# xuyuan/waymo_2d_tracking

Hardware: AMD Instinct MI355X
Metric: end-to-end frames/sec (detect+SORT) on 1920x1280 Waymo frames (higher is better)
Workload: dtype f32; 1 GPU; Cascade R-CNN X152-32x8d-FPN dconv (random-init, fp32, batch 1) on synthetic 1920x1280x3 frames -> top-100 detections/frame -> SORT (max_age 2, min_hits 0, all boxes tracked; trackers resident for the whole segment); 5 cameras x 2 frames per step per GPU; 1x1 and dense 3x3 convolutions: f32 operands as exact 3 x bf16 splits, six cross terms on the bf16 matrix cores, f32 accumulate (csrc/det_gemm_s; stage=e2e, parallelism=sequence-shard x1

## Files before the change

### include/waymodet.h

```cpp
#ifndef WAYMODET_H
#define WAYMODET_H
#include <stddef.h>
#include <stdint.h>
#ifdef __cplusplus
extern "C" {
#endif

int wd_roi_pool_fpn_f32(const float* const* feats, const int32_t* heights, const int32_t* widths,
                        const float* scales, int n_levels, int channels, int batch,
                        const float* rois, int n_rois, int pooled, int min_level, int canonical_level,
                        float canonical_size, float* out, void* stream);

size_t wd_nms_workspace(int n);
int wd_select_kept(const uint8_t* keep_mask, const uint8_t* valid, const int64_t* order, int n, int cap, int64_t* out_idx,
                   int32_t* count, void* stream);
int wd_nms_sorted_f32(const float* boxes, const int32_t* idxs, int n, float iou_threshold,
                      uint8_t* keep_mask, int32_t* n_keep, void* workspace, size_t workspace_bytes, void* stream);

size_t wd_gemm_nt_workspace(int M, int N, int K);
int wd_gemm_nt_ws_f32(const float* A, const float* Bt, const float* bias, const float* residual, int relu, int M, int N, int K,
                      float* C, void* workspace, size_t workspace_bytes, void* stream);

int wd_gemm_lt_f32(const float* a, const float* w, const float* bias, const float* residual, float* out, int m, int n, int k,
                   int relu, void* workspace, size_t workspace_bytes, void* stream);
int wd_gemm_lt_plan_info(int m, int n, int k, int relu, int has_bias, int has_residual, float* best_us, int* candidates);
size_t wd_gemm_split_packed_bytes(int N, int K);
int wd_gemm_split_pack_weight(const float* w, int N, int K, void* packed, void* stream);
int wd_gemm_split_pack_weight_strided(const float* w, int N, int K, long stride_n, long stride_k, void* packed, void* stream);
typedef struct WdSplitPackDesc {
    const float* src;
    void* dst;
    long s_n, s_c, s_kh, s_kw;
    long first_block;
    int N, K, C, ksize, flip, reserved;
} WdSplitPackDesc;
int wd_gemm_split_pack_batch(const WdSplitPackDesc* descs_device, int count, long total_blocks, void* stream);
size_t wd_gemm_split_workspace(long M, int N, int K);
int wd_gemm_split_f32(const float* a, long lda, const void* packed_w, const float* bias, const float* residual, float* out, long ldc,
                      int M, int N, int K, int relu, void* workspace, size_t workspace_bytes, void* stream);
int wd_conv_split_f32(const float* x, int batch, int H, int W, int C, const void* packed_w, int ksize, int stride, int pad, const float* bias,
                      const float* residual, float* out, int N, int relu, void* workspace, size_t workspace_bytes, void* stream);
int wd_gemm_split_supported(const float* a, long lda, const float* bias, const float* residual, const float* out, long ldc, long M, int N, int K);
int wd_conv_split_position_major(int batch, int H, int W, int ksize, int stride, int pad);
typedef struct WdSplitIO {
    const float* a;
    long lda;
    const void* a_planes;
    const float* residual;
    const void* residual_planes;
    float* out;
    void* out_planes;
    long ldc;
} WdSplitIO;
size_t wd_split_planes_bytes(long M, int K);
int wd_split_planes_pack_f32(const float* a, long lda, long M, int K, void* planes, void* stream);
int wd_split_planes_unpack_f32(const void* planes, long M, int K, float* out, long ldo, void* stream);
int wd_gemm_split_io(const WdSplitIO* io, const void* packed_w, const float* bias, int M, int N, int K, int relu, void* workspace,
                     size_t workspace_bytes, void* stream);
int wd_nms_segmented_f32(const float* boxes, const int32_t* idxs, const int32_t* seg_offsets, int n_seg, float iou_threshold,
                         uint8_t* keep_mask, int32_t* n_keep, void* workspace, size_t workspace_bytes, void* stream);

size_t wd_rpn_topk_workspace(const int* n_per_level, int n_levels, int k);
int wd_rpn_topk_decode_f32(const float* const* logits, const float* const* deltas, const float* const* anchors,
                           const int* n_per_level, int n_levels, int k, float img_h, float img_w, float scale_clamp,
                           float* out_boxes, float* out_scores, int32_t* out_group, uint8_t* out_valid, void* workspace,
                           size_t workspace_bytes, void* stream);
int wd_sort_candidates_f32(const float* boxes, const float* scores, const int32_t* group, const uint8_t* valid,
                           const uint8_t* valid2 , int n, float* out_boxes, float* out_scores, int32_t* out_group, uint8_t* out_valid, int64_t* out_order,
                           void* stream);
int wd_box_candidates_f32(const float* boxes, const float* s0, const float* s1, const float* s2, const int32_t* n_valid, int rows,
                          int num_classes, float score_thresh, float img_h, float img_w, float* out_boxes, float* out_scores,
                          int32_t* out_group, uint8_t* out_valid, int64_t* out_order, void* stream);
int wd_gather_kept_f32(const uint8_t* keep, const uint8_t* valid, const float* boxes, const float* scores, const int64_t* order,
                       int n, int cap, int num_classes, float* out_boxes, float* out_scores, int64_t* out_class, int32_t* count,
                       void* stream);
int wd_detections_to_wire(const float* boxes, const float* scores, const int64_t* classes, const int32_t* count, int n, int in_w,
                          int in_h, int hflip, int out_w, int out_h, double* xywhs, int32_t* category, void* stream);

size_t wd_deform_packed_weight_floats(int c_in, int c_out, int groups);
int wd_deform_pack_weight(const float* weight_oihw, int c_in, int c_out, int groups, float* packed, void* stream);
const char* wd_deform_conv3x3_variant(int c_in, int groups, int stride, int pad, int has_offset);
const char* wd_deform_conv3x3_last_kernel(void);
int wd_deform_conv3x3_f32(const float* x, const float* offset, const float* mask, const float* packed_weight,
                          const float* scale, const float* bias, int relu,
                          int batch, int h, int w, int c_in, int c_out, int groups, int stride, int pad,
                          float* y, void* stream);
int wd_deform_conv3x3_hint_f32(const float* x, const float* offset, const float* mask, const float* packed_weight,
                               const float* scale, const float* bias, int relu, int batch, int h, int w, int c_in,
                               int c_out, int groups, int stride, int pad, int far_offsets, float* y, void* stream);
size_t wd_deform_table_bytes(int batch, int h, int w);
int wd_deform_offsets_table_f32(const float* partial, int ld, const float* bias, int batch, int h, int w, float* offsets,
                                void* table, void* stream);
int wd_deform_conv3x3_tab_f32(const float* x, const float* offset, const float* mask, const float* packed_weight,
                              const float* scale, const float* bias, int relu, int batch, int h, int w, int c_in,
                              int c_out, int groups, int stride, int pad, int far_offsets, const void* table, float* y,
                              void* stream);

int wd_gemm_nt_f32(const float* A, const float* Bt, const float* bias, const float* residual, int relu,
                   int M, int N, int K, float* C, void* stream);

int wd_groupnorm_relu_nhwc_f32(float* x, const float* gamma, const float* beta, int n, int hw, int c, int groups,
                               float eps, int relu, void* stream);
int wd_groupnorm_relu_out_nhwc_f32(const float* x, float* y, const float* gamma, const float* beta, int n, int hw, int c, int groups,
                                   float eps, int relu, void* stream);
int wd_groupnorm_relu_bwd_nhwc_f32(const float* x, const float* dy, const float* gamma, const float* beta, int n, int hw, int c, int groups,
                                   float eps, int relu, float* dx, float* dgamma, float* dbeta, void* stream);

#define WD_LAYOUT_NCHW_F32 0
#define WD_LAYOUT_NHWC_U8 1
int wd_preprocess_out_shape(int h, int w, double scale, int divisor, int* ho, int* wo, int* hp, int* wp);
int wd_preprocess_f32(const void* src, int src_layout, int batch, int h, int w, double scale, int hflip, int vflip,
                      int swap_rb, const float* mean3, const float* std3, int divisor, float* out, void* stream);

int wd_decode_boxes_f32(const float* deltas, const float* boxes, const int64_t* index, int n, float wx, float wy, float ww,
                        float wh, float scale_clamp, float clip_w, float clip_h, float* out, void* stream);

int wd_roi_pool_fpn_bwd_f32(float* const* grad_feats, const int32_t* heights, const int32_t* widths, const float* scales,
                            int n_levels, int channels, int batch, const float* rois, int n_rois, int pooled, int min_level,
                            int canonical_level, float canonical_size, const float* grad_out, void* stream);
int wd_deform_im2col_f32(const float* x, const float* offset, int batch, int h, int w, int c, int groups, int stride, int pad,
                         float* col, void* stream);
int wd_deform_col2im_f32(const float* dcol, const float* x, const float* offset, int batch, int h, int w, int c, int groups,
                         int stride, int pad, float* dx, float* doffset, void* stream);
size_t wd_deform_bwd_tables_bytes(int batch, int h, int w, int stride);
int wd_deform_dxoff_f32(const float* x, const float* offset, const float* dy, const float* y_act, const float* scale, const float* weight, int batch,
                        int h, int w, int c, int groups, int stride, unsigned char* tables, float* packed_weight, float* dx, float* doffset,
                        void* stream);
size_t wd_deform_dw_scratch_floats(int batch, int h, int w, int c, int groups, int stride);
int wd_deform_dw_f32(const float* x, const float* offset, const float* dy, const float* y_act, const float* scale, int batch, int h, int w, int c,
                     int groups, int stride, float* scratch, float* dw, void* stream);

int wd_tap_shift_add_f32(const float* partial, int ld, int n_out, const float* bias, int batch, int h, int w, int stride,
                         float* out, void* stream);

int wd_upsample2x_nhwc_f32(const float* src, int batch, int h, int w, int c, float* dst, void* stream);

int wd_bias_relu_f32(float* y, const float* bias, long m, int n, int relu, void* stream);

int wd_act_bwd_f32(const float* dy, const float* y, const float* scale, long m, int n, int relu, float* g, void* stream);

int wd_autocontrast_u8(uint8_t* img, int h, int w, void* workspace24, void* stream);

int wd_jpeg_info(const uint8_t* data, int64_t n, int32_t* width, int32_t* height, int32_t* components, int32_t* h_samp,
                 int32_t* v_samp, int32_t* restart_interval);
int wd_jpeg_decode_rgb_u8(const uint8_t* data, int64_t n, uint8_t* rgb, int64_t capacity, int32_t* width, int32_t* height,
                          int32_t* sync_rounds, void* stream);
int wd_jpeg_last_stats(int32_t* out4);

#ifdef __cplusplus
}
#endif
#endif
```

### waymo_2d_tracking_amd/csrc/det_deform.hip

```cpp
#include "common.h"
#include "../../include/waymodet.h"
#include <cstdlib>

namespace {

using f32x4 = __attribute__((ext_vector_type(4))) float;
constexpr int TP = 64;
constexpr int CCH = 128;
constexpr int LDC = CCH + 2;

struct Sample {
    unsigned idx[4];
    float wgt[4];
};

template <int CG, bool DEFORM>
__global__ __launch_bounds__(256, (CG <= 32 ? 3 : 2)) void deform_conv3x3_kernel(
    const float* __restrict__ x, const float* __restrict__ offset, const float* __restrict__ mask,
    const float* __restrict__ wp, const float* __restrict__ scale, const float* __restrict__ bias, int relu,
    int batch, int H, int W, int C, int Cout, int Ho, int Wo, int stride, int pad, float* __restrict__ y) {
    constexpr bool PRIV = CG <= 32;
    constexpr int LDW = PRIV ? 34 : LDC;
    __shared__ Sample tab[TP * 9];
    __shared__ __attribute__((aligned(16))) float col[PRIV ? 4 * TP * 34 : TP * LDC];
    const int tid = threadIdx.x, lane = tid & 63, wave = tid >> 6;
    const int tiles_x = (Wo + 7) >> 3, tiles_y = (Ho + 7) >> 3;
    const int ntiles = batch * tiles_y * tiles_x;
    const int nchunks = C / CCH;
    int tile, chunk;
    {
        const int b = blockIdx.x;
        const int xcd = b & 7, slot = b >> 3;
        if (nchunks >= 8 && (nchunks & 7) == 0) {
            const int cpx = nchunks >> 3;
            chunk = xcd * cpx + slot % cpx;
            tile = slot / cpx;
        } else if (nchunks < 8 && (8 % nchunks) == 0 && (ntiles % (8 / nchunks)) == 0) {
            const int xpc = 8 / nchunks;
            const int tpp = ntiles / xpc;
            chunk = xcd / xpc;
            tile = (xcd % xpc) * tpp + slot;
        } else {
            chunk = b / ntiles;
            tile = b - chunk * ntiles;
        }
    }
    if (tile >= ntiles || chunk >= nchunks) return;
    const int tn = tile / (tiles_y * tiles_x);
    const int trem = tile - tn * tiles_y * tiles_x;
    const int tyy = trem / tiles_x, txx = trem - tyy * tiles_x;
    __shared__ int pix[TP];
    if (tid < TP) {
        const int ho = tyy * 8 + (tid >> 3), wo = txx * 8 + (tid & 7);
        pix[tid] = (ho < Ho && wo < Wo) ? (tn * Ho + ho) * Wo + wo : -1;
    }
    __syncthreads();
    const int c0 = chunk * CCH;
    for (int e = tid; e < TP * 9; e += 256) {
        const int p = e / 9, k = e - 9 * p;
        const long gp = pix[p];
        Sample s;
#pragma unroll
        for (int q = 0; q < 4; ++q) { s.idx[q] = 0u; s.wgt[q] = 0.f; }
        if (gp >= 0) {
            const int n = (int)(gp / ((long)Ho * Wo));
            const int rem = (int)(gp - (long)n * Ho * Wo);
            const int ho = rem / Wo, wo = rem - ho * Wo;
            const int kh = k / 3, kw = k - 3 * kh;
            if (!DEFORM) {
                const int hi = ho * stride - pad + kh, wi = wo * stride - pad + kw;
                if (hi >= 0 && hi < H && wi >= 0 && wi < W) { s.idx[0] = (unsigned)(n * H * W + hi * W + wi) * (unsigned)C * 4u; s.wgt[0] = 1.f; }
                tab[e] = s;
                continue;
            }
            const float* off = offset + (size_t)gp * 18;
            const float h_im = (float)(ho * stride - pad + kh) + off[2 * k];
            const float w_im = (float)(wo * stride - pad + kw) + off[2 * k + 1];
            if (h_im > -1.f && w_im > -1.f && h_im < (float)H && w_im < (float)W) {
                const int hl = (int)floorf(h_im), wl = (int)floorf(w_im);
                const int hh = hl + 1, wh = wl + 1;
                const float lh = h_im - (float)hl, lw = w_im - (float)wl;
                const float uh = 1.f - lh, uw = 1.f - lw;
                const float m = mask ? mask[(size_t)gp * 9 + k] : 1.f;
                const int base = n * H * W;
                if (hl >= 0 && wl >= 0) { s.idx[0] = (unsigned)(base + hl * W + wl) * (unsigned)C * 4u; s.wgt[0] = uh * uw * m; }
                if (hl >= 0 && wh <= W - 1) { s.idx[1] = (unsigned)(base + hl * W + wh) * (unsigned)C * 4u; s.wgt[1] = uh * lw * m; }
                if (hh <= H - 1 && wl >= 0) { s.idx[2] = (unsigned)(base + hh * W + wl) * (unsigned)C * 4u; s.wgt[2] = lh * uw * m; }
                if (hh <= H - 1 && wh <= W - 1) { s.idx[3] = (unsigned)(base + hh * W + wh) * (unsigned)C * 4u; s.wgt[3] = lh * lw * m; }
            }
        }
        tab[e] = s;
    }
    f32x4 acc[4][2];
#pragma unroll
    for (int i = 0; i < 4; ++i)
#pragma unroll
        for (int j = 0; j < 2; ++j) acc[i][j] = (f32x4){0.f, 0.f, 0.f, 0.f};
    __syncthreads();

    const int gq = PRIV ? (lane & 7) : (tid & 31);
    const int gp0 = PRIV ? (lane >> 3) : (tid >> 5);
    const int co_w = wave * 32;
    float* colw = PRIV ? col + wave * (TP * 34) : col;
    auto slab_sync = [&]() {
        if (PRIV) {
            __builtin_amdgcn_fence(__ATOMIC_RELEASE, "wavefront");
            __builtin_amdgcn_wave_barrier();
            __builtin_amdgcn_fence(__ATOMIC_ACQUIRE, "wavefront");
        } else {
            __syncthreads();
        }
    };
    constexpr int NQ = DEFORM ? 4 : 1;
    const char* xb = reinterpret_cast<const char*>(x);
    const unsigned lane_off = (unsigned)(c0 + (PRIV ? co_w : 0) + gq * 4) * 4u;
    float4 tA[4][NQ];
    auto issue = [&](int k, int half, float4 (&t)[4][NQ]) {
#pragma unroll
        for (int i = 0; i < 4; ++i) {
            const int p = gp0 + 8 * (half * 4 + i);
            const Sample& s = tab[p * 9 + k];
#pragma unroll
            for (int q = 0; q < NQ; ++q)
                t[i][q] = *reinterpret_cast<const float4*>(xb + (size_t)(s.idx[q] + lane_off));
        }
    };
    auto blend = [&](int k, int half, const float4 (&t)[4][NQ]) {
#pragma unroll
        for (int i = 0; i < 4; ++i) {
            const int p = gp0 + 8 * (half * 4 + i);
            const Sample& s = tab[p * 9 + k];
            float4 v = make_float4(0.f, 0.f, 0.f, 0.f);
#pragma unroll
            for (int q = 0; q < NQ; ++q) {
                const float wq = s.wgt[q];
                v.x += wq * t[i][q].x; v.y += wq * t[i][q].y;
                v.z += wq * t[i][q].z; v.w += wq * t[i][q].w;
            }
            float2* d = reinterpret_cast<float2*>(&colw[p * LDW + gq * 4]);
            d[0] = make_float2(v.x, v.y);
            d[1] = make_float2(v.z, v.w);
        }
    };
    constexpr int KS = (CG >= 16) ? CG / 4 : 4;
    float bR[2][KS];
    auto load_b = [&](int k) {
#pragma unroll
        for (int nt = 0; nt < 2; ++nt) {
            const int co_l = co_w + 16 * nt;
            if (CG >= 16) {
                const int g = (c0 + co_l) / CG;
                const int co_g = (co_l % CG) + (lane & 15);
                const float* wb = wp + ((size_t)(g * 9 + k) * CG) * CG + co_g;
#pragma unroll
                for (int kk = 0; kk < KS; ++kk) bR[nt][kk] = wb[(size_t)(kk * 4 + (lane >> 4)) * CG];
            } else {
                const int j = lane & 15;
                const int g = (c0 + co_l) / 8 + (j >> 3);
#pragma unroll
                for (int kk = 0; kk < KS; ++kk) {
                    const int ci = kk * 4 + (lane >> 4);
                    const float wv = wp[((size_t)(g * 9 + k) * 8 + (ci & 7)) * 8 + (j & 7)];
                    bR[nt][kk] = ((ci >> 3) == (j >> 3)) ? wv : 0.f;
                }
            }
        }
    };
    issue(0, 0, tA);
    for (int k = 0; k < 9; ++k) {
        blend(k, 0, tA);
        load_b(k);
        {
            float4 tB[4][NQ];
            issue(k, 1, tB);
            __builtin_amdgcn_sched_barrier(0);
            blend(k, 1, tB);
        }
        slab_sync();
        if (k + 1 < 9) issue(k + 1, 0, tA);
        __builtin_amdgcn_sched_barrier(0);
#pragma unroll
        for (int nt = 0; nt < 2; ++nt) {
            const int co_l = co_w + 16 * nt;
            const int cl = PRIV ? 16 * nt : co_l;
            const int a_col = (CG >= 16) ? (cl / CG) * CG : cl;
#pragma unroll
            for (int kk = 0; kk < KS; ++kk) {
                const int ci = kk * 4 + (lane >> 4);
#pragma unroll
                for (int mt = 0; mt < 4; ++mt) {
                    const float a = colw[(mt * 16 + (lane & 15)) * LDW + a_col + ci];
                    acc[mt][nt] = __builtin_amdgcn_mfma_f32_16x16x4f32(a, bR[nt][kk], acc[mt][nt], 0, 0, 0);
                }
            }
        }
        slab_sync();
    }
#pragma unroll
    for (int nt = 0; nt < 2; ++nt) {
        const int co = c0 + co_w + 16 * nt + (lane & 15);
        const float sc = scale ? scale[co] : 1.f;
        const float bi = bias ? bias[co] : 0.f;
#pragma unroll
        for (int mt = 0; mt < 4; ++mt)
#pragma unroll
            for (int r = 0; r < 4; ++r) {
                const long gp = pix[mt * 16 + (lane >> 4) * 4 + r];
                if (gp >= 0) {
                    float v = acc[mt][nt][r] * sc + bi;
                    if (relu) v = fmaxf(v, 0.f);
                    y[(size_t)gp * Cout + co] = v;
                }
            }
    }
}


constexpr int PCH = 64;
constexpr int PR = 2;
constexpr int PS = 10 + 2 * PR;
constexpr int LDP = PCH + 2;

template <int CG>
__global__ __launch_bounds__(256, 2) void deform_conv3x3_patch_kernel(
    const float* __restrict__ x, const float* __restrict__ offset, const float* __restrict__ mask,
    const float* __restrict__ wp, const float* __restrict__ scale, const float* __restrict__ bias, int relu,
    int batch, int H, int W, int C, int Cout, int Ho, int Wo, float* __restrict__ y) {
    __shared__ __attribute__((aligned(16))) float patch[PS * PS * PCH];
    __shared__ __attribute__((aligned(16))) float col[TP * LDP];
    __shared__ float offs[TP * 18];
    __shared__ float msk[TP * 9];
    __shared__ int pix[TP];
    const int tid = threadIdx.x, lane = tid & 63, wave = tid >> 6;
    const int tiles_x = (Wo + 7) >> 3, tiles_y = (Ho + 7) >> 3;
    const int ntiles = batch * tiles_y * tiles_x;
    const int nchunks = C / PCH;
    int tile, chunk;
    {
        const int b = blockIdx.x;
        const int xcd = b & 7, slot = b >> 3;
        if ((nchunks & 7) == 0) {
            const int cpx = nchunks >> 3;
            chunk = xcd * cpx + slot % cpx;
            tile = slot / cpx;
        } else {
            chunk = b / ntiles;
            tile = b - chunk * ntiles;
        }
    }
    if (tile >= ntiles || chunk >= nchunks) return;
    const int tn = tile / (tiles_y * tiles_x);
    const int trem = tile - tn * tiles_y * tiles_x;
    const int tyy = trem / tiles_x, txx = trem - tyy * tiles_x;
    const int c0 = chunk * PCH;
    const int py0 = tyy * 8 - 1 - PR, px0 = txx * 8 - 1 - PR;
    if (tid < TP) {
        const int ho = tyy * 8 + (tid >> 3), wo = txx * 8 + (tid & 7);
        pix[tid] = (ho < Ho && wo < Wo) ? (tn * Ho + ho) * Wo + wo : -1;
    }
    for (int e = tid; e < PS * PS * (PCH / 4); e += 256) {
        const int pp = e >> 4, q = e & 15;
        const int r = pp / PS, cc = pp - r * PS;
        const int iy = py0 + r, ix = px0 + cc;
        float4 v = make_float4(0.f, 0.f, 0.f, 0.f);
        if (iy >= 0 && iy < H && ix >= 0 && ix < W)
            v = *reinterpret_cast<const float4*>(x + ((size_t)(tn * H + iy) * W + ix) * C + c0 + q * 4);
        *reinterpret_cast<float4*>(&patch[pp * PCH + q * 4]) = v;
    }
    __syncthreads();
    for (int e = tid; e < TP * 18; e += 256) {
        const int p = e / 18;
        const int gp = pix[p];
        offs[e] = gp >= 0 ? offset[(size_t)gp * 18 + (e - 18 * p)] : 0.f;
    }
    for (int e = tid; e < TP * 9; e += 256) {
        const int p = e / 9;
        const int gp = pix[p];
        msk[e] = (gp >= 0) ? (mask ? mask[(size_t)gp * 9 + (e - 9 * p)] : 1.f) : 0.f;
    }
    f32x4 acc[4];
#pragma unroll
    for (int i = 0; i < 4; ++i) acc[i] = (f32x4){0.f, 0.f, 0.f, 0.f};
    __syncthreads();

    const int gq = tid & 15;
    const int gp0 = tid >> 4;
    const int co_l = wave * 16;
    const int g_l = co_l / CG;
    const int g = (c0 + co_l) / CG;
    const int co_g = (co_l % CG) + (lane & 15);
    for (int k = 0; k < 9; ++k) {
        const int kh = k / 3, kw = k - 3 * kh;
        float breg[CG / 4];
        {
            const float* wb = wp + ((size_t)(g * 9 + k) * CG) * CG + co_g;
#pragma unroll
            for (int kk = 0; kk < CG / 4; ++kk) breg[kk] = wb[(size_t)(kk * 4 + (lane >> 4)) * CG];
        }
#pragma unroll
        for (int i = 0; i < 4; ++i) {
            const int p = gp0 + 16 * i;
            const float ry = (float)((p >> 3) + kh + PR) + offs[p * 18 + 2 * k];
            const float rx = (float)((p & 7) + kw + PR) + offs[p * 18 + 2 * k + 1];
            const float h_im = ry + (float)py0, w_im = rx + (float)px0;
            const float m = msk[p * 9 + k];
            float4 v = make_float4(0.f, 0.f, 0.f, 0.f);
            if (m != 0.f && h_im > -1.f && w_im > -1.f && h_im < (float)H && w_im < (float)W) {
                const float fy = floorf(ry), fx = floorf(rx);
                const int hl = (int)fy, wl = (int)fx;
                const float lh = ry - fy, lw = rx - fx, uh = 1.f - lh, uw = 1.f - lw;
                if (hl >= 0 && hl < PS - 1 && wl >= 0 && wl < PS - 1) {
                    const float* pb = &patch[(hl * PS + wl) * PCH + gq * 4];
                    const float4 a = *reinterpret_cast<const float4*>(pb);
                    const float4 b = *reinterpret_cast<const float4*>(pb + PCH);
                    const float4 c = *reinterpret_cast<const float4*>(pb + PS * PCH);
                    const float4 d = *reinterpret_cast<const float4*>(pb + PS * PCH + PCH);
                    const float w1 = uh * uw, w2 = uh * lw, w3 = lh * uw, w4 = lh * lw;
                    v.x = w1 * a.x + w2 * b.x + w3 * c.x + w4 * d.x;
                    v.y = w1 * a.y + w2 * b.y + w3 * c.y + w4 * d.y;
                    v.z = w1 * a.z + w2 * b.z + w3 * c.z + w4 * d.z;
                    v.w = w1 * a.w + w2 * b.w + w3 * c.w + w4 * d.w;
                } else {
                    const int ih = hl + py0, iw = wl + px0;
                    const float wq[4] = {uh * uw, uh * lw, lh * uw, lh * lw};
#pragma unroll
                    for (int qd = 0; qd < 4; ++qd) {
                        const int yy = ih + (qd >> 1), xx = iw + (qd & 1);
                        if (yy >= 0 && yy < H && xx >= 0 && xx < W) {
                            const float4 t = *reinterpret_cast<const float4*>(x + ((size_t)(tn * H + yy) * W + xx) * C + c0 + gq * 4);
                            v.x += wq[qd] * t.x; v.y += wq[qd] * t.y; v.z += wq[qd] * t.z; v.w += wq[qd] * t.w;
                        }
                    }
                }
                v.x *= m; v.y *= m; v.z *= m; v.w *= m;
            }
            float2* dd = reinterpret_cast<float2*>(&col[p * LDP + gq * 4]);
            dd[0] = make_float2(v.x, v.y);
            dd[1] = make_float2(v.z, v.w);
        }
        __syncthreads();
#pragma unroll
        for (int kk = 0; kk < CG / 4; ++kk) {
            const int ci = kk * 4 + (lane >> 4);
#pragma unroll
            for (int mt = 0; mt < 4; ++mt) {
                const float a = col[(mt * 16 + (lane & 15)) * LDP + g_l * CG + ci];
                acc[mt] = __builtin_amdgcn_mfma_f32_16x16x4f32(a, breg[kk], acc[mt], 0, 0, 0);
            }
        }
        __syncthreads();
    }
    const int co = c0 + co_l + (lane & 15);
    const float sc = scale ? scale[co] : 1.f;
    const float bi = bias ? bias[co] : 0.f;
#pragma unroll
    for (int mt = 0; mt < 4; ++mt)
#pragma unroll
        for (int r = 0; r < 4; ++r) {
            const long gp = pix[mt * 16 + (lane >> 4) * 4 + r];
            if (gp >= 0) {
                float v = acc[mt][r] * sc + bi;
                if (relu) v = fmaxf(v, 0.f);
                y[(size_t)gp * Cout + co] = v;
            }
        }
}

#define PROW(p) (((p) >> 4) + 4 * (((p) >> 3) & 1))
constexpr int PST = PCH + 4;
template <int CG>
__global__ __launch_bounds__(256, 2) void deform_conv3x3_lds_kernel(
    const float* __restrict__ x, const float* __restrict__ offset, const float* __restrict__ mask,
    const float* __restrict__ wp, const float* __restrict__ scale, const float* __restrict__ bias, int relu,
    int batch, int H, int W, int C, int Cout, int Ho, int Wo, float* __restrict__ y) {
    constexpr int GPW = PCH / CG;
    constexpr int WPG = 4 / GPW;
    constexpr int MT = 4 / WPG;
    constexpr int NT = CG / 16;
    constexpr int KS = CG / 4;
    constexpr int PW = 16 * MT;
    __shared__ __attribute__((aligned(16))) float patch[PS * PS * PST];
    __shared__ __attribute__((aligned(16))) float4 tw[TP * 9];
    __shared__ int toff[TP * 9];
    __shared__ int pix[TP];
    __shared__ int any_fb;
    const int tid = threadIdx.x, lane = tid & 63, wave = tid >> 6;
    const int tiles_x = (Wo + 7) >> 3, tiles_y = (Ho + 7) >> 3;
    const int ntiles = batch * tiles_y * tiles_x;
    const int nchunks = C / PCH;
    int tile, chunk;
    {
        const int b = blockIdx.x;
        const int xcd = b & 7, slot = b >> 3;
        if ((nchunks & 7) == 0) {
            const int cpx = nchunks >> 3;
            chunk = xcd * cpx + slot % cpx;
            tile = slot / cpx;
        } else {
            chunk = b / ntiles;
            tile = b - chunk * ntiles;
        }
    }
    if (tile >= ntiles || chunk >= nchunks) return;
    const int tn = tile / (tiles_y * tiles_x);
    const int trem = tile - tn * tiles_y * tiles_x;
    const int tyy = trem / tiles_x, txx = trem - tyy * tiles_x;
    const int c0 = chunk * PCH;
    const int py0 = tyy * 8 - 1 - PR, px0 = txx * 8 - 1 - PR;
    if (tid == 0) any_fb = 0;
    if (tid < TP) {
        const int ho = tyy * 8 + PROW(tid), wo = txx * 8 + (tid & 7);
        pix[tid] = (ho < Ho && wo < Wo) ? (tn * Ho + ho) * Wo + wo : -1;
    }
    const int g_l = wave / WPG;
    const int p_base = (wave % WPG) * PW;
    const int r16 = lane & 15, kq = lane >> 4;
    const int ch_l = g_l * CG + kq * KS;
    const int g = (c0 + g_l * CG) / CG;
    float bR[2][NT][KS];
    const float* __restrict__ wfrag = wp + (size_t)Cout * CG * 9 + ((size_t)g * 9 * 64 + lane) * (NT * KS);
    auto load_b = [&](int k, float (&b)[NT][KS]) {
        const float4* src = reinterpret_cast<const float4*>(wfrag + (size_t)k * 64 * (NT * KS));
#pragma unroll
        for (int j = 0; j < NT * KS / 4; ++j) {
            const float4 v = src[j];
            b[(4 * j) / KS][(4 * j) % KS + 0] = v.x; b[(4 * j) / KS][(4 * j) % KS + 1] = v.y;
            b[(4 * j) / KS][(4 * j) % KS + 2] = v.z; b[(4 * j) / KS][(4 * j) % KS + 3] = v.w;
        }
    };
    load_b(0, bR[0]);
    constexpr int NE = (TP * 9 + 255) / 256;
    float e_dy[NE], e_dx[NE], e_m[NE];
    int e_gp[NE];
#pragma unroll
    for (int j = 0; j < NE; ++j) {
        const int e = tid + 256 * j;
        const int p = e / 9, k = e - 9 * p;
        int gp = -1;
        if (e < TP * 9) {
            const int ho = tyy * 8 + PROW(p), wo = txx * 8 + (p & 7);
            gp = (ho < Ho && wo < Wo) ? (tn * Ho + ho) * Wo + wo : -1;
        }
        e_gp[j] = gp;
        e_dy[j] = e_dx[j] = 0.f;
        e_m[j] = 1.f;
        if (gp >= 0) {
            e_dy[j] = offset[(size_t)gp * 18 + 2 * k];
            e_dx[j] = offset[(size_t)gp * 18 + 2 * k + 1];
            if (mask) e_m[j] = mask[(size_t)gp * 9 + k];
        }
    }
    {
        constexpr int NL = (PS * PS * (PCH / 4) + 255) / 256;
        float4 v[NL];
#pragma unroll
        for (int j = 0; j < NL; ++j) {
            const int e = tid + 256 * j;
            const int pp = e >> 4, q = e & 15;
            const int r = pp / PS, cc = pp - r * PS;
            const int iy = py0 + r, ix = px0 + cc;
            v[j] = make_float4(0.f, 0.f, 0.f, 0.f);
            if (e < PS * PS * (PCH / 4) && iy >= 0 && iy < H && ix >= 0 && ix < W)
                v[j] = *reinterpret_cast<const float4*>(x + ((size_t)(tn * H + iy) * W + ix) * C + c0 + q * 4);
        }
#pragma unroll
        for (int j = 0; j < NL; ++j) {
            const int e = tid + 256 * j;
            if (e < PS * PS * (PCH / 4)) *reinterpret_cast<float4*>(&patch[(e >> 4) * PST + (e & 15) * 4]) = v[j];
        }
    }
    __syncthreads();
#pragma unroll
    for (int j = 0; j < NE; ++j) {
        const int e = tid + 256 * j;
        if (e >= TP * 9) continue;
        const int p = e / 9, k = e - 9 * p;
        float4 w4 = make_float4(0.f, 0.f, 0.f, 0.f);
        int off = 0;
        if (e_gp[j] >= 0) {
            const int kh = k / 3, kw = k - 3 * kh;
            const float ry = (float)(PROW(p) + kh + PR) + e_dy[j];
            const float rx = (float)((p & 7) + kw + PR) + e_dx[j];
            const float h_im = ry + (float)py0, w_im = rx + (float)px0;
            const float m = e_m[j];
            if (h_im > -1.f && w_im > -1.f && h_im < (float)H && w_im < (float)W) {
                const float fy = floorf(ry), fx = floorf(rx);
                const int hl = (int)fy, wl = (int)fx;
                const float lh = ry - fy, lw = rx - fx, uh = 1.f - lh, uw = 1.f - lw;
                w4 = make_float4(uh * uw * m, uh * lw * m, lh * uw * m, lh * lw * m);
                if (hl >= 0 && hl < PS - 1 && wl >= 0 && wl < PS - 1) {
                    off = (hl * PS + wl) * PST;
                } else {
                    off = -1 - ((hl + py0 + 2) * (W + 4) + (wl + px0 + 2));
                    any_fb = 1;
                }
            }
        }
        tw[e] = w4;
        toff[e] = off;
    }
    f32x4 acc[MT][NT];
#pragma unroll
    for (int i = 0; i < MT; ++i)
#pragma unroll
        for (int j = 0; j < NT; ++j) acc[i][j] = (f32x4){0.f, 0.f, 0.f, 0.f};
    __syncthreads();
    const bool slow = any_fb != 0;

    auto mfma = [&](const float (&a)[MT][KS], const float (&b)[NT][KS]) {
#pragma unroll
        for (int kk = 0; kk < KS; ++kk) {
#pragma unroll
            for (int mt = 0; mt < MT; ++mt)
#pragma unroll
                for (int nt = 0; nt < NT; ++nt)
                    acc[mt][nt] = __builtin_amdgcn_mfma_f32_16x16x4f32(a[mt][kk], b[nt][kk], acc[mt][nt], 0, 0, 0);
        }
    };
    if (!slow) {
        float4 cv[MT][4][KS / 4];
        float4 wv[MT];
        float a[2][MT][KS];
        auto gather_issue = [&](int k) {
#pragma unroll
            for (int mt = 0; mt < MT; ++mt) {
                const int e = (p_base + mt * 16 + r16) * 9 + k;
                const float* pb = &patch[toff[e] + ch_l];
                wv[mt] = tw[e];
#pragma unroll
                for (int h = 0; h < KS / 4; ++h) {
                    cv[mt][0][h] = *reinterpret_cast<const float4*>(pb + 4 * h);
                    cv[mt][1][h] = *reinterpret_cast<const float4*>(pb + PST + 4 * h);
                    cv[mt][2][h] = *reinterpret_cast<const float4*>(pb + PS * PST + 4 * h);
                    cv[mt][3][h] = *reinterpret_cast<const float4*>(pb + PS * PST + PST + 4 * h);
                }
            }
        };
        auto blend = [&](float (&o)[MT][KS]) {
#pragma unroll
            for (int mt = 0; mt < MT; ++mt)
#pragma unroll
                for (int h = 0; h < KS / 4; ++h) {
                    o[mt][4 * h + 0] = wv[mt].x * cv[mt][0][h].x + wv[mt].y * cv[mt][1][h].x + wv[mt].z * cv[mt][2][h].x + wv[mt].w * cv[mt][3][h].x;
                    o[mt][4 * h + 1] = wv[mt].x * cv[mt][0][h].y + wv[mt].y * cv[mt][1][h].y + wv[mt].z * cv[mt][2][h].y + wv[mt].w * cv[mt][3][h].y;
                    o[mt][4 * h + 2] = wv[mt].x * cv[mt][0][h].z + wv[mt].y * cv[mt][1][h].z + wv[mt].z * cv[mt][2][h].z + wv[mt].w * cv[mt][3][h].z;
                    o[mt][4 * h + 3] = wv[mt].x * cv[mt][0][h].w + wv[mt].y * cv[mt][1][h].w + wv[mt].z * cv[mt][2][h].w + wv[mt].w * cv[mt][3][h].w;
                }
        };
        gather_issue(0);
        blend(a[0]);
#pragma unroll
        for (int k = 0; k < 9; ++k) {
            if (k + 1 < 9) load_b(k + 1, bR[(k + 1) & 1]);
            if (k + 1 < 9) gather_issue(k + 1);
            mfma(a[k & 1], bR[k & 1]);
            if (k + 1 < 9) blend(a[(k + 1) & 1]);
            if (k + 1 < 9) {
                constexpr int NM = MT * NT * KS;
                constexpr int NDS = MT * (2 + KS);
                constexpr int H1 = NM / 4;
                __builtin_amdgcn_sched_group_barrier(0x020, NT * KS / 4, 0);
#pragma unroll
                for (int j = 0; j < H1; ++j) {
                    __builtin_amdgcn_sched_group_barrier(0x008, 1, 0);
                    __builtin_amdgcn_sched_group_barrier(0x100, (NDS + H1 - 1) / H1, 0);
                }
#pragma unroll
                for (int j = 0; j < NM / 4; ++j) __builtin_amdgcn_sched_group_barrier(0x008, 1, 0);
#pragma unroll
                for (int j = 0; j < NM - H1 - NM / 4; ++j) {
                    __builtin_amdgcn_sched_group_barrier(0x008, 1, 0);
                    __builtin_amdgcn_sched_group_barrier(0x002, (MT * KS * 4 + (NM - H1 - NM / 4) - 1) / (NM - H1 - NM / 4), 0);
                }
            }
            __builtin_amdgcn_sched_barrier(0);
        }
    } else {
#pragma unroll
        for (int k = 0; k < 9; ++k) {
            if (k + 1 < 9) load_b(k + 1, bR[(k + 1) & 1]);
            float a[MT][KS];
#pragma unroll
            for (int mt = 0; mt < MT; ++mt) {
                const int e = (p_base + mt * 16 + r16) * 9 + k;
                const int off = toff[e];
                const float4 w4 = tw[e];
                const float wq[4] = {w4.x, w4.y, w4.z, w4.w};
#pragma unroll
                for (int kk = 0; kk < KS; ++kk) a[mt][kk] = 0.f;
                if (off >= 0) {
                    const float* pb = &patch[off + ch_l];
#pragma unroll
                    for (int qd = 0; qd < 4; ++qd)
#pragma unroll
                        for (int h = 0; h < KS / 4; ++h) {
                            const float4 t = *reinterpret_cast<const float4*>(pb + (qd >> 1) * PS * PST + (qd & 1) * PST + 4 * h);
                            a[mt][4 * h + 0] += wq[qd] * t.x; a[mt][4 * h + 1] += wq[qd] * t.y;
                            a[mt][4 * h + 2] += wq[qd] * t.z; a[mt][4 * h + 3] += wq[qd] * t.w;
                        }
                } else {
                    const int code = -1 - off;
                    const int ih = code / (W + 4) - 2, iw = code - (ih + 2) * (W + 4) - 2;
#pragma unroll
                    for (int qd = 0; qd < 4; ++qd) {
                        const int yy = ih + (qd >> 1), xx = iw + (qd & 1);
                        if (yy >= 0 && yy < H && xx >= 0 && xx < W) {
                            const float* gb = x + ((size_t)(tn * H + yy) * W + xx) * C + c0 + ch_l;
#pragma unroll
                            for (int h = 0; h < KS / 4; ++h) {
                                const float4 t = *reinterpret_cast<const float4*>(gb + 4 * h);
                                a[mt][4 * h + 0] += wq[qd] * t.x; a[mt][4 * h + 1] += wq[qd] * t.y;
                                a[mt][4 * h + 2] += wq[qd] * t.z; a[mt][4 * h + 3] += wq[qd] * t.w;
                            }
                        }
                    }
                }
            }
            mfma(a, bR[k & 1]);
        }
    }
#pragma unroll
    for (int nt = 0; nt < NT; ++nt) {
        const int co = c0 + g_l * CG + 16 * nt + (lane & 15);
        const float sc = scale ? scale[co] : 1.f;
        const float bi = bias ? bias[co] : 0.f;
#pragma unroll
        for (int mt = 0; mt < MT; ++mt)
#pragma unroll
            for (int r = 0; r < 4; ++r) {
                const long gp = pix[p_base + mt * 16 + (lane >> 4) * 4 + r];
                if (gp >= 0) {
                    float v = acc[mt][nt][r] * sc + bi;
                    if (relu) v = fmaxf(v, 0.f);
                    y[(size_t)gp * Cout + co] = v;
                }
            }
    }
}

__global__ void pack_weight_kernel(const float* __restrict__ w, int cg, int cout, float* __restrict__ packed) {
    const long total = (long)cout * cg * 9;
    for (long e = (long)blockIdx.x * blockDim.x + threadIdx.x; e < total; e += (long)gridDim.x * blockDim.x) {
        const int co = (int)(e % cg);
        const int ci = (int)((e / cg) % cg);
        const int k = (int)((e / ((long)cg * cg)) % 9);
        const int g = (int)(e / ((long)cg * cg * 9));
        const float v = w[(((size_t)(g * cg + co) * cg) + ci) * 9 + k];
        packed[e] = v;
        if (cg == 16 || cg == 32) {
            const int KS = cg / 4, NT = cg / 16;
            const int kq = ci / KS, kk = ci - kq * KS, nt = co >> 4, r16 = co & 15;
            const int lane = kq * 16 + r16;
            packed[total + (((size_t)(g * 9 + k) * 64 + lane) * NT + nt) * KS + kk] = v;
        }
    }
}

}

int wt::victim_regs_deform64() {
    hipFuncAttributes at{};
    if (hipFuncGetAttributes(&at, reinterpret_cast<const void*>(deform_conv3x3_kernel<64, true>)) != hipSuccess) return 0;
    return (at.numRegs + 7) / 8 * 8;
}


int wd_deform_pp_launch(const float* x, const float* offset, const float* packed_weight, const float* scale,
                        const float* bias, int relu, int batch, int h, int w, int c, int cg, int stride, hipStream_t stream, float* y,
                        const void* table);
int wd_grouped_conv3x3_c8_launch(const float* x, const float* packed_weight, const float* scale, const float* bias, int relu,
                                 int batch, int h, int w, int c, hipStream_t stream, float* y);

static int deform_variant(int cg, int stride, int pad, bool has_offset, const char* mode) {
    const bool fits = has_offset && stride == 1 && pad == 1;
    if (mode && strcmp(mode, "none") == 0) return 0;
    if (has_offset && stride == 2 && pad == 1 && (cg == 32 || cg == 16) && !(mode && strcmp(mode, "lds") == 0)) return 3;
    if (mode && strcmp(mode, "all") == 0) return (fits && (cg == 16 || cg == 32 || cg == 64)) ? 1 : 0;
    if (fits && (cg == 32 || cg == 16) && !(mode && strcmp(mode, "lds") == 0)) return 3;
    if (fits && (cg == 16 || cg == 32)) return 2;
    if (fits && cg == 64) return 1;
    return 0;
}

static const char* variant_kernel_name(int variant, int cg, bool has_offset) {
    switch (variant) {
        case 3: return cg == 16 ? "deform_conv3x3_pp_kernel<16>" : "deform_conv3x3_pp_kernel<32>";
        case 2: return cg == 16 ? "deform_conv3x3_lds_kernel<16>" : "deform_conv3x3_lds_kernel<32>";
        case 1: return cg == 16 ? "deform_conv3x3_patch_kernel<16>" : cg == 32 ? "deform_conv3x3_patch_kernel<32>" : "deform_conv3x3_patch_kernel<64>";
        default: break;
    }
    if (has_offset) return cg == 8 ? "deform_conv3x3_kernel<8,true>" : cg == 16 ? "deform_conv3x3_kernel<16,true>" : cg == 32 ? "deform_conv3x3_kernel<32,true>" : "deform_conv3x3_kernel<64,true>";
    return cg == 8 ? "deform_conv3x3_kernel<8,false>" : cg == 16 ? "deform_conv3x3_kernel<16,false>" : cg == 32 ? "deform_conv3x3_kernel<32,false>" : "deform_conv3x3_kernel<64,false>";
}

static thread_local const char* last_kernel = "";

extern "C" {

const char* wd_deform_conv3x3_variant(int c_in, int groups, int stride, int pad, int has_offset) {
    if (groups <= 0 || c_in % groups) return "invalid";
    const int cg = c_in / groups;
    const int variant = deform_variant(cg, stride, pad, has_offset != 0, getenv("WD_DEFORM_PATCH"));
    if (variant == 0 && !has_offset && cg == 8 && stride == 1 && pad == 1 && (c_in % 128) == 0) return "grouped_conv3x3_c8_kernel";
    return variant_kernel_name(variant, cg, has_offset != 0);
}

const char* wd_deform_conv3x3_last_kernel(void) { return last_kernel; }

size_t wd_deform_packed_weight_floats(int c_in, int c_out, int groups) {
    if (groups <= 0 || c_in % groups || c_in != c_out) return 0;
    return 2 * (size_t)c_out * (size_t)(c_in / groups) * 9;
}

int wd_deform_pack_weight(const float* weight_oihw, int c_in, int c_out, int groups, float* packed, void* stream) {
    WT_TRY(wt::ensure_device());
    if (!wd_deform_packed_weight_floats(c_in, c_out, groups)) {
        wt::set_error("wd_deform_pack_weight: needs c_in == c_out divisible by groups");
        return WT_ERR_INVALID;
    }
    hipLaunchKernelGGL(pack_weight_kernel, dim3(256), dim3(256), 0, (hipStream_t)stream, weight_oihw, c_in / groups, c_out, packed);
    WT_HIP(hipGetLastError());
    return WT_OK;
}

int wd_deform_conv3x3_f32(const float* x, const float* offset, const float* mask, const float* packed_weight,
                          const float* scale, const float* bias, int relu, int batch, int h, int w, int c_in,
                          int c_out, int groups, int stride, int pad, float* y, void* stream_) {
    return wd_deform_conv3x3_tab_f32(x, offset, mask, packed_weight, scale, bias, relu, batch, h, w, c_in, c_out, groups, stride, pad,
                                     0, nullptr, y, stream_);
}

int wd_deform_conv3x3_hint_f32(const float* x, const float* offset, const float* mask, const float* packed_weight,
                               const float* scale, const float* bias, int relu, int batch, int h, int w, int c_in,
                               int c_out, int groups, int stride, int pad, int far_offsets, float* y, void* stream_) {
    return wd_deform_conv3x3_tab_f32(x, offset, mask, packed_weight, scale, bias, relu, batch, h, w, c_in, c_out, groups, stride, pad,
                                     far_offsets, nullptr, y, stream_);
}

int wd_deform_conv3x3_tab_f32(const float* x, const float* offset, const float* mask, const float* packed_weight,
                              const float* scale, const float* bias, int relu, int batch, int h, int w, int c_in,
                              int c_out, int groups, int stride, int pad, int far_offsets, const void* table, float* y,
                              void* stream_) {
    WT_TRY(wt::ensure_device());
    if (c_in != c_out || groups <= 0 || c_in % groups || c_in % CCH || stride < 1 || batch < 1 || h < 1 || w < 1 ||
        ((uintptr_t)x & 15)) {
        wt::set_error("wd_deform_conv3x3_f32: unsupported shape (c_in=%d c_out=%d groups=%d; need c_in == c_out, c_in %% 128 == 0)",
                      c_in, c_out, groups);
        return WT_ERR_INVALID;
    }
    if ((double)batch * h * w * c_in * 4.0 >= 4294967296.0) {
        wt::set_error("wd_deform_conv3x3_f32: input of %d x %d x %d x %d floats exceeds the kernel's 32-bit byte offsets (4 GiB); "
                      "split the batch", batch, h, w, c_in);
        return WT_ERR_CAPACITY;
    }
    const int cg = c_in / groups;
    const int ho = (h + 2 * pad - 3) / stride + 1, wo = (w + 2 * pad - 3) / stride + 1;
    if (ho < 1 || wo < 1) return WT_OK;
    const long ntiles = (long)batch * ((ho + 7) / 8) * ((wo + 7) / 8);
    const long nwg = ntiles * (c_in / CCH);
    dim3 grid((unsigned)((nwg + 7) / 8 * 8));
    hipStream_t stream = (hipStream_t)stream_;
    const char* mode = getenv("WD_DEFORM_PATCH");
    last_kernel = "";
    if (!offset && !mask && cg == 8 && stride == 1 && pad == 1 && (c_in % 128) == 0 && ((uintptr_t)y & 7) == 0) {
        last_kernel = "grouped_conv3x3_c8_kernel";
        return wd_grouped_conv3x3_c8_launch(x, packed_weight, scale, bias, relu, batch, h, w, c_in, stream, y);
    }
    int variant = deform_variant(cg, stride, pad, offset != nullptr, mode);
    if (variant == 3 && stride != 1 && mask) variant = 0;
    if (variant == 3 && stride == 1 && (mask || far_offsets)) variant = 2;
    if (cg == 8 || cg == 16 || cg == 32 || cg == 64) last_kernel = variant_kernel_name(variant, cg, offset != nullptr);
    if (variant == 3)
        return wd_deform_pp_launch(x, offset, packed_weight, scale, bias, relu, batch, h, w, c_in, cg, stride, stream, y, table);
    if (variant == 2) {
        const long nwg_p = ntiles * (c_in / PCH);
        dim3 gridp((unsigned)((nwg_p + 7) / 8 * 8));
        if (cg == 16)
            hipLaunchKernelGGL(deform_conv3x3_lds_kernel<16>, gridp, dim3(256), 0, stream, x, offset, mask, packed_weight, scale,
                               bias, relu, batch, h, w, c_in, c_out, ho, wo, y);
        else
            hipLaunchKernelGGL(deform_conv3x3_lds_kernel<32>, gridp, dim3(256), 0, stream, x, offset, mask, packed_weight, scale,
                               bias, relu, batch, h, w, c_in, c_out, ho, wo, y);
        WT_HIP(hipGetLastError());
        return WT_OK;
    }
    if (variant == 1) {
        const long nwg_p = ntiles * (c_in / PCH);
        dim3 gridp((unsigned)((nwg_p + 7) / 8 * 8));
#define WD_LAUNCH_P(CG)                                                                                              \
    hipLaunchKernelGGL(deform_conv3x3_patch_kernel<CG>, gridp, dim3(256), 0, stream, x, offset, mask, packed_weight, \
                       scale, bias, relu, batch, h, w, c_in, c_out, ho, wo, y)
        if (cg == 16) WD_LAUNCH_P(16);
        else if (cg == 32) WD_LAUNCH_P(32);
        else WD_LAUNCH_P(64);
#undef WD_LAUNCH_P
        WT_HIP(hipGetLastError());
        return WT_OK;
    }
#define WD_LAUNCH(CG)                                                                                                     \
    do {                                                                                                                  \
        if (offset)                                                                                                       \
            hipLaunchKernelGGL((deform_conv3x3_kernel<CG, true>), grid, dim3(256), 0, stream, x, offset, mask,           \
                               packed_weight, scale, bias, relu, batch, h, w, c_in, c_out, ho, wo, stride, pad, y);       \
        else                                                                                                              \
            hipLaunchKernelGGL((deform_conv3x3_kernel<CG, false>), grid, dim3(256), 0, stream, x, offset, mask,          \
                               packed_weight, scale, bias, relu, batch, h, w, c_in, c_out, ho, wo, stride, pad, y);       \
    } while (0)
    if (cg == 16) WD_LAUNCH(16);
    else if (cg == 32) WD_LAUNCH(32);
    else if (cg == 64) WD_LAUNCH(64);
    else if (cg == 8) WD_LAUNCH(8);
    else {
        wt::set_error("wd_deform_conv3x3_f32: channels per group must be 8, 16, 32 or 64 (got %d)", cg);
        return WT_ERR_INVALID;
    }
#undef WD_LAUNCH
    WT_HIP(hipGetLastError());
    return WT_OK;
}

}
```

### waymo_2d_tracking_amd/csrc/det_deform_pp.hip

```cpp
#include <cstdlib>
#include <mutex>
#include <vector>
#include <type_traits>
#include "common.h"
#include "../../include/waymodet.h"

namespace {

using f32x4 = __attribute__((ext_vector_type(4))) float;
using f32x2 = __attribute__((ext_vector_type(2))) float;
using u32x4 = __attribute__((ext_vector_type(4))) unsigned;

#ifndef PP_SPLIT32
#define PP_SPLIT32 0
#endif
namespace pp {
constexpr int PS = 14;
constexpr int NPIX = PS * PS;
constexpr int CH = 32;
constexpr int PATCH_F = (NPIX + 1) * CH;
constexpr int PATCH_B = PATCH_F * 4;
constexpr int NE = 64 * 9;
constexpr int TAB_B = NE * 16;
constexpr unsigned FAR_Y = 0xFFFFFFFFu;
#ifndef PP_RES_TAPS
#define PP_RES_TAPS 3
#endif
constexpr int RW = PP_RES_TAPS;
template <int CG> constexpr int tap_floats() { return (CG == 32 ? 4 : 2) * 64 * 4; }
constexpr int NT = 2;
template <int CG> constexpr size_t smem_bytes() { return (size_t)(9 - RW) * tap_floats<CG>() * 4 + 2 * NT * (size_t)PATCH_B + 2 * NT * (size_t)TAB_B; }
}

#ifdef PP_NO_BARRIER
#define PP_BARRIER() do { asm volatile("" ::: "memory"); } while (0)
#else
#define PP_BARRIER() do { asm volatile("" ::: "memory"); __builtin_amdgcn_s_barrier(); asm volatile("" ::: "memory"); } while (0)
#endif
#define PP_SLOT() do { asm volatile("" ::: "memory"); __builtin_amdgcn_sched_barrier(0); } while (0)

__device__ __forceinline__ int pp_row_pixel(int r, int m) {
    const int blk = r >> 2, i = r & 3;
    const int y = m + 4 * (blk >> 1);
    const int x = 2 * i + ((blk == 1 || blk == 2) ? 1 : 0);
    return y * 8 + x;
}

__device__ __forceinline__ int pp_slot(int p, int q) { return (p << 3) + (q ^ ((p >> 1) & 7)); }

__device__ __forceinline__ int pp_origin(int stride) { return stride == 1 ? 3 : -1; }

__device__ __forceinline__ uint4 pp_make_entry(bool pixel_in_image, int yy, int xx, int kh, int kw, float2 ov, int ty, int tx, int H, int W,
                                               int stride) {
    constexpr int ps = pp::PS;
    const int org = pp_origin(stride);
    const float t_fy = (float)(stride * yy + kh - 1 + org), t_fx = (float)(stride * xx + kw - 1 + org);
    const float py0 = (float)(ty * 8 * stride - org), px0 = (float)(tx * 8 * stride - org);
    const float fH = (float)H, fW = (float)W;
    unsigned s0 = pp_slot(ps * ps, 0), s1 = s0, s2 = s0, s3 = s0;
    float lh = 0.f, lw = 0.f;
    uint4 e;
    if (pixel_in_image) {
        const float ry = t_fy + ov.x, rx = t_fx + ov.y;
        const float h_im = ry + py0, w_im = rx + px0;
        if (h_im > -1.f && w_im > -1.f && h_im < fH && w_im < fW) {
            const float fy = floorf(ry), fx = floorf(rx);
            const int hl = (int)fy, wl = (int)fx;
            lh = ry - fy; lw = rx - fx;
            if ((unsigned)hl <= (unsigned)(ps - 2) && (unsigned)wl <= (unsigned)(ps - 2)) {
                const int u = hl * ps + wl;
                s0 = pp_slot(u, 0); s1 = pp_slot(u + 1, 0); s2 = pp_slot(u + ps, 0); s3 = pp_slot(u + ps + 1, 0);
            } else {
                const int ih = hl + ty * 8 * stride - org, iw = wl + tx * 8 * stride - org;
                e.x = (unsigned)(ih + 32768) | ((unsigned)(iw + 32768) << 16);
                e.y = pp::FAR_Y;
                e.z = __float_as_uint(lh); e.w = __float_as_uint(lw);
                return e;
            }
        }
    }
    e.x = (s0 << 4) | (s1 << 20); e.y = (s2 << 4) | (s3 << 20);
    e.z = __float_as_uint(lh); e.w = __float_as_uint(lw);
    return e;
}

__device__ __forceinline__ void pp_tile_flag(bool far, int tile, int ntiles, uint4* __restrict__ table) {
    const int any = __syncthreads_or(far ? 1 : 0);
    if (threadIdx.x == 0) reinterpret_cast<unsigned*>(table + (size_t)ntiles * pp::NE)[tile] = any ? 1u : 0u;
}

__global__ __launch_bounds__(576) void deform_offsets_table_kernel(const float* __restrict__ partial, int ld,
                                                                  const float* __restrict__ bias, int batch, int H, int W,
                                                                  float* __restrict__ offsets, uint4* __restrict__ table) {
    const int tiles_x = (W + 7) >> 3, tiles_y = (H + 7) >> 3;
    const int ntiles = batch * tiles_y * tiles_x;
    for (int t = blockIdx.x; t < ntiles; t += gridDim.x) {
        const int e = threadIdx.x;
        int tile = t;
        const int tx = tile % tiles_x;
        tile /= tiles_x;
        const int ty = tile % tiles_y, tn = tile / tiles_y;
        const int pxl = e / 9, k = e - 9 * pxl;
        const int yy = pxl >> 3, xx = pxl & 7, kh = k / 3, kw = k - 3 * kh;
        const int oy = ty * 8 + yy, ox = tx * 8 + xx;
        const bool in = oy < H && ox < W;
        float2 ov = make_float2(0.f, 0.f);
        if (in) {
            float a0 = bias ? bias[2 * k] : 0.f, a1 = bias ? bias[2 * k + 1] : 0.f;
            const float* base = partial + (size_t)tn * H * W * ld + 2 * k;
#pragma unroll
            for (int qh = 0; qh < 3; ++qh) {
                const int y = oy + qh - 1;
                if (y < 0 || y >= H) continue;
#pragma unroll
                for (int qw = 0; qw < 3; ++qw) {
                    const int x = ox + qw - 1;
                    if (x < 0 || x >= W) continue;
                    const float2 v = *reinterpret_cast<const float2*>(base + ((size_t)y * W + x) * ld + (qh * 3 + qw) * 18);
                    a0 += v.x; a1 += v.y;
                }
            }
            ov = make_float2(a0, a1);
            *reinterpret_cast<float2*>(offsets + (((size_t)tn * H + oy) * W + ox) * 18 + 2 * k) = ov;
        }
        const uint4 ent = pp_make_entry(in, yy, xx, kh, kw, ov, ty, tx, H, W, 1);
        table[(size_t)t * pp::NE + e] = ent;
        pp_tile_flag(ent.y == pp::FAR_Y, t, ntiles, table);
    }
}

__global__ __launch_bounds__(576) void deform_table_kernel(const float* __restrict__ offsets, int batch, int Hin, int Win, int H, int W,
                                                          int stride, uint4* __restrict__ table) {
    const int tiles_x = (W + 7) >> 3, tiles_y = (H + 7) >> 3;
    const int ntiles = batch * tiles_y * tiles_x;
    for (int t = blockIdx.x; t < ntiles; t += gridDim.x) {
        const int e = threadIdx.x;
        int tile = t;
        const int tx = tile % tiles_x;
        tile /= tiles_x;
        const int ty = tile % tiles_y, tn = tile / tiles_y;
        const int pxl = e / 9, k = e - 9 * pxl;
        const int yy = pxl >> 3, xx = pxl & 7, kh = k / 3, kw = k - 3 * kh;
        const int oy = ty * 8 + yy, ox = tx * 8 + xx;
        const bool in = oy < H && ox < W;
        float2 ov = make_float2(0.f, 0.f);
        if (in) ov = *reinterpret_cast<const float2*>(offsets + (((size_t)tn * H + oy) * W + ox) * 18 + 2 * k);
        const uint4 ent = pp_make_entry(in, yy, xx, kh, kw, ov, ty, tx, Hin, Win, stride);
        table[(size_t)t * pp::NE + e] = ent;
        pp_tile_flag(ent.y == pp::FAR_Y, t, ntiles, table);
    }
}

template <int CG>
__global__ __launch_bounds__(256 * pp::NT, pp::NT) __attribute__((amdgpu_waves_per_eu(pp::NT, pp::NT))) void deform_conv3x3_pp_kernel(
    const float* __restrict__ x, const float* __restrict__ wfrag, const float* __restrict__ scale, const float* __restrict__ bias,
    int relu, int batch, int H, int W, int Ho, int Wo, int stride, int C, int Cout, int nsplit, float* __restrict__ y,
    const uint4* __restrict__ table) {
    static_assert(CG == 32 || CG == 16, "32 channels per group, or two groups of 16 per item");
    constexpr int NQ = CG == 32 ? 4 : 2;
    constexpr int RW = pp::RW, NT = pp::NT;
    constexpr int PS = pp::PS, NPIX = pp::NPIX;
    constexpr int PATCH_F = pp::PATCH_F, PATCH_B = pp::PATCH_B;
    constexpr int NPC = (NPIX * 8 + 255) / 256;
    static_assert((NPIX + 1) * 8 * 16 <= 65536, "corner byte offsets are 16 bits");
    extern __shared__ __attribute__((aligned(16))) char smem[];
    float* bw = reinterpret_cast<float*>(smem);
    constexpr unsigned PATCH0 = (unsigned)((9 - RW) * pp::tap_floats<CG>() * 4);
    constexpr unsigned TAB0 = PATCH0 + 2u * NT * PATCH_B;
    const int tid = threadIdx.x, lane = tid & 63;
    const int wave = __builtin_amdgcn_readfirstlane(tid >> 6);
    const int team = wave >> 2, m = wave & 3;
    const int r16 = lane & 15, kq = lane >> 4;
    const int tiles_x = (Wo + 7) >> 3, tiles_y = (Ho + 7) >> 3;
    const int ntiles = batch * tiles_y * tiles_x;
    const int org = pp_origin(stride), tstep = 8 * stride;
    const int g = blockIdx.x / nsplit, sidx = blockIdx.x - g * nsplit;
    const int tq = ntiles / nsplit, trm = ntiles - tq * nsplit;
    const int t0 = sidx * tq + (sidx < trm ? sidx : trm);
    const int t1 = t0 + tq + (sidx < trm ? 1 : 0);
    const int n_items = (t1 - t0 + NT - 1) / NT;
    const unsigned patch_b0 = PATCH0 + (unsigned)team * 2u * PATCH_B;
    const unsigned tab_b0 = TAB0 + (unsigned)team * 2u * pp::TAB_B;
    const int c0 = g * pp::CH;
    const long HW = (long)H * W, HWo = (long)Ho * Wo;
    const char* xb = reinterpret_cast<const char*>(x);

    int p_rel[NPC], p_rc[NPC];
#pragma unroll
    for (int j = 0; j < NPC; ++j) {
        const int sl = (NPC * m + j) * 64 + lane;
        const int pxl = sl >> 3, q = (sl & 7) ^ ((pxl >> 1) & 7);
        const int r = pxl / PS, cc = pxl - r * PS;
        p_rel[j] = ((r * W + cc) * C + q * 4) * 4;
        p_rc[j] = (sl < NPIX * 8) ? ((r << 8) | cc) : 0xFFFF;
    }

    struct TileXY { int tn, ty, tx; };
    auto tile_of = [&](int t) {
        TileXY r;
        r.tn = t / (tiles_y * tiles_x);
        const int trem = t - r.tn * tiles_y * tiles_x;
        const int band = trem / (2 * tiles_x), rb = trem - band * 2 * tiles_x;
        if (2 * band + 1 < tiles_y) { r.tx = rb >> 1; r.ty = 2 * band + (rb & 1); }
        else { r.tx = rb; r.ty = 2 * band; }
        return r;
    };
    auto tile_xy = [&](int it) {
        int t = t0 + team + NT * it;
        t = t < t1 ? t : t1 - 1;
        return tile_of(t);
    };
    auto tile_valid = [&](int it) { return t0 + team + NT * it < t1; };

    auto dma16 = [&](const char* sbase, int voff, unsigned dst) {
        unsigned keep;
        asm volatile("s_mov_b32 %0, m0\n\ts_mov_b32 m0, %3\n\ts_nop 0\n\tglobal_load_lds_dwordx4 %1, %2\n\ts_mov_b32 m0, %0"
                     : "=&s"(keep) : "v"(voff), "s"(sbase), "s"(dst) : "memory");
    };
    auto issue_patch = [&](const TileXY& T, unsigned base) {
        const int py0 = T.ty * tstep - org, px0 = T.tx * tstep - org;
        const char* pbase = xb + (((long)T.tn * HW + (long)py0 * W + px0) * C + c0) * 4;
        const bool inner = py0 >= 0 && px0 >= 0 && py0 + PS <= H && px0 + PS <= W;
        if (inner) {
#pragma unroll
            for (int j = 0; j < NPC; ++j) {
                const int s0 = (NPC * m + j) * 64;
                if (s0 + 64 <= NPIX * 8) dma16(pbase, p_rel[j], base + s0 * 16);
                else if (s0 < NPIX * 8) { if (p_rc[j] != 0xFFFF) dma16(pbase, p_rel[j], base + s0 * 16); }
            }
            return;
        }
        float* pb = reinterpret_cast<float*>(smem + base);
#pragma unroll
        for (int j = 0; j < NPC; ++j) {
            const int s0 = (NPC * m + j) * 64;
            if (s0 >= NPIX * 8) continue;
            const int iy = py0 + (p_rc[j] >> 8), ix = px0 + (p_rc[j] & 255);
            const bool in = p_rc[j] != 0xFFFF && iy >= 0 && iy < H && ix >= 0 && ix < W;
            if (in) {
                const char* src = pbase + p_rel[j];
                unsigned keep;
                const unsigned dst = base + s0 * 16;
                asm volatile("s_mov_b32 %0, m0\n\ts_mov_b32 m0, %2\n\ts_nop 0\n\tglobal_load_lds_dwordx4 %1, off\n\ts_mov_b32 m0, %0"
                             : "=&s"(keep) : "v"(src), "s"(dst) : "memory");
            } else if (p_rc[j] != 0xFFFF) {
                *reinterpret_cast<float4*>(pb + (s0 + lane) * 4) = make_float4(0.f, 0.f, 0.f, 0.f);
            }
        }
    };
    const int tab_voff = lane * 16;
    auto issue_table = [&](const TileXY& T, unsigned tbase) {
        const char* tb = reinterpret_cast<const char*>(table) + ((size_t)(T.tn * tiles_y + T.ty) * tiles_x + T.tx) * pp::TAB_B;
#pragma unroll
        for (int i = 0; i < 3; ++i) {
            const int piece = m + 4 * i;
            if (piece < 9) dma16(tb + piece * 1024, tab_voff, tbase + piece * 1024);
        }
    };

    f32x4 wres[RW > 0 ? RW : 1][NQ];
    float4 aff_sc[2], aff_bi[2];
    {
        if constexpr (CG == 32) {
            const f32x4* src = reinterpret_cast<const f32x4*>(wfrag + (size_t)g * 9 * 64 * 16);
            for (int e = tid; e < (9 - RW) * 64 * 4; e += 256 * NT) {
                const int j = e & 3, ln = (e >> 2) & 63, k = e >> 8;
                *reinterpret_cast<f32x4*>(bw + ((k * 4 + j) * 64 + ln) * 4) = src[e + RW * 256];
            }
#pragma unroll
            for (int k = 0; k < RW; ++k)
#pragma unroll
                for (int j = 0; j < NQ; ++j) wres[k][j] = src[(k * 64 + lane) * 4 + j];
        } else {
            const f32x4* src = reinterpret_cast<const f32x4*>(wfrag + (size_t)(2 * g) * 9 * 64 * 4);
            for (int e = tid; e < (9 - RW) * 2 * 64; e += 256 * NT) {
                const int ln = e & 63, j = (e >> 6) & 1, k = e >> 7;
                *reinterpret_cast<f32x4*>(bw + ((k * 2 + j) * 64 + ln) * 4) = src[(j * 9 + k + RW) * 64 + ln];
            }
#pragma unroll
            for (int k = 0; k < RW; ++k)
#pragma unroll
                for (int j = 0; j < NQ; ++j) wres[k][j] = src[(j * 9 + k) * 64 + lane];
        }
#pragma unroll
        for (int nt = 0; nt < 2; ++nt) {
            const int c = c0 + 16 * nt + 4 * kq;
            aff_sc[nt] = scale ? *reinterpret_cast<const float4*>(scale + c) : make_float4(1.f, 1.f, 1.f, 1.f);
            aff_bi[nt] = bias ? *reinterpret_cast<const float4*>(bias + c) : make_float4(0.f, 0.f, 0.f, 0.f);
        }
        if (tid < 2 * NT * pp::CH)
            reinterpret_cast<float*>(smem + PATCH0)[(tid >> 5) * PATCH_F + NPIX * pp::CH + (tid & 31)] = 0.f;
        const TileXY T0 = tile_xy(0);
        issue_patch(T0, patch_b0);
        issue_table(T0, tab_b0);
        __builtin_amdgcn_s_waitcnt(0x0F70);
    }
    f32x4 acc[4], done[2];
    const int my_p = pp_row_pixel(r16, m);
    const int my_y = my_p >> 3, my_x = my_p & 7;

    TileXY prev = {0, 0, 0};
    bool prev_valid = false;
    auto epilogue = [&]() {
        if (!prev_valid) return;
        const int ho = prev.ty * 8 + my_y, wo = prev.tx * 8 + my_x;
        if (ho < Ho && wo < Wo) {
            float* dst = y + ((long)prev.tn * HWo + (long)ho * Wo + wo) * Cout + c0 + 4 * kq;
#pragma unroll
            for (int nt = 0; nt < 2; ++nt) {
                const float4 sc = aff_sc[nt], bi = aff_bi[nt];
                float4 v;
                v.x = done[nt][0] * sc.x + bi.x; v.y = done[nt][1] * sc.y + bi.y;
                v.z = done[nt][2] * sc.z + bi.z; v.w = done[nt][3] * sc.w + bi.w;
                if (relu) { v.x = fmaxf(v.x, 0.f); v.y = fmaxf(v.y, 0.f); v.z = fmaxf(v.z, 0.f); v.w = fmaxf(v.w, 0.f); }
                *reinterpret_cast<float4*>(dst + 16 * nt) = v;
            }
        }
    };

    float a[8];
    f32x4 b[2][NQ];
    f32x4 cv[8];
    float w00 = 0.f, w01 = 0.f, w10 = 0.f, w11 = 0.f;
    bool far_nxt = false;
    unsigned ad0 = 0, ad1 = 0, ad2 = 0, ad3 = 0;
    u32x4 ent = {0u, 0u, 0u, 0u};
    constexpr unsigned QX = CG == 32 ? 16u : 64u;
    const unsigned kx = (unsigned)(CG == 32 ? 2 * kq : kq) << 4;
    const int my_ch = (CG == 32 ? 8 * kq : 4 * kq);
    const unsigned my_ent = (unsigned)(my_p * 9) * 16u;
    using lds4 = const __attribute__((address_space(3))) f32x4*;
    using ldsu4 = const __attribute__((address_space(3))) u32x4*;

    auto read_entry = [&](unsigned tbase, int k) { ent = *(ldsu4)(uintptr_t)(tbase + my_ent + (unsigned)k * 16u); };
    auto prep = [&](unsigned base) {
        const float lh = __uint_as_float(ent.z), lw = __uint_as_float(ent.w);
        const float uh = 1.f - lh, uw = 1.f - lw;
        w00 = uh * uw; w01 = uh * lw; w10 = lh * uw; w11 = lh * lw;
        far_nxt = ent.y == pp::FAR_Y;
        ad0 = ((ent.x & 0xFFFFu) ^ kx) + base;
        ad1 = ((ent.x >> 16) ^ kx) + base;
        ad2 = ((ent.y & 0xFFFFu) ^ kx) + base;
        ad3 = ((ent.y >> 16) ^ kx) + base;
#ifdef PP_LIN_CORNER
        ad0 = base + lane * 32; ad1 = ad0 + 2048; ad2 = ad0 + 4096; ad3 = ad0 + 6144;
#endif
    };
    auto lds_corners = [&]() {
        cv[0] = *(lds4)(uintptr_t)ad0; cv[1] = *(lds4)(uintptr_t)(ad0 ^ QX);
        cv[2] = *(lds4)(uintptr_t)ad1; cv[3] = *(lds4)(uintptr_t)(ad1 ^ QX);
        cv[4] = *(lds4)(uintptr_t)ad2; cv[5] = *(lds4)(uintptr_t)(ad2 ^ QX);
        cv[6] = *(lds4)(uintptr_t)ad3; cv[7] = *(lds4)(uintptr_t)(ad3 ^ QX);
    };
    auto issue_reads = [&](auto FARC, int k, f32x4 (&bb)[NQ], bool want_w, int tn) {
        constexpr bool FAR = decltype(FARC)::value;
#ifndef PP_NO_FAR
        if (FAR && __builtin_expect(__ballot(far_nxt) != 0, 0)) {
            if (far_nxt) {
                const int ih = (int)(ent.x & 0xFFFFu) - 32768, iw = (int)(ent.x >> 16) - 32768;
                const bool y0 = ih >= 0 && ih < H, y1 = ih + 1 >= 0 && ih + 1 < H, x0 = iw >= 0 && iw < W, x1 = iw + 1 >= 0 && iw + 1 < W;
                w00 = (y0 && x0) ? w00 : 0.f; w01 = (y0 && x1) ? w01 : 0.f; w10 = (y1 && x0) ? w10 : 0.f; w11 = (y1 && x1) ? w11 : 0.f;
                const int ya = min(max(ih, 0), H - 1), yb = min(max(ih + 1, 0), H - 1);
                const int xa = min(max(iw, 0), W - 1), xc = min(max(iw + 1, 0), W - 1);
                const char* gb = reinterpret_cast<const char*>(x + (long)tn * HW * C + c0);
                constexpr unsigned Q2 = CG == 32 ? 16u : 64u;
                const unsigned ch_b = (unsigned)my_ch * 4u, rowa = (unsigned)(ya * W), rowb = (unsigned)(yb * W), cb = (unsigned)C * 4u;
                const unsigned o00 = (rowa + (unsigned)xa) * cb + ch_b, o01 = (rowa + (unsigned)xc) * cb + ch_b;
                const unsigned o10 = (rowb + (unsigned)xa) * cb + ch_b, o11 = (rowb + (unsigned)xc) * cb + ch_b;
                cv[0] = *reinterpret_cast<const f32x4*>(gb + o00); cv[1] = *reinterpret_cast<const f32x4*>(gb + (o00 + Q2));
                cv[2] = *reinterpret_cast<const f32x4*>(gb + o01); cv[3] = *reinterpret_cast<const f32x4*>(gb + (o01 + Q2));
                cv[4] = *reinterpret_cast<const f32x4*>(gb + o10); cv[5] = *reinterpret_cast<const f32x4*>(gb + (o10 + Q2));
                cv[6] = *reinterpret_cast<const f32x4*>(gb + o11); cv[7] = *reinterpret_cast<const f32x4*>(gb + (o11 + Q2));
            } else {
                lds_corners();
            }
        } else
#endif
        {
            lds_corners();
        }
        if (want_w) {
#pragma unroll
            for (int j = 0; j < NQ; ++j) bb[j] = *(lds4)(uintptr_t)((unsigned)(((k - RW) * NQ + j) * 1024) + (unsigned)lane * 16u);
        }
    };
    auto blend = [&]() {
#ifdef PP_NO_BLEND
        a[0] = cv[0].x; a[1] = cv[1].y; a[2] = cv[2].x; a[3] = cv[3].y; a[4] = cv[4].x; a[5] = cv[5].x; a[6] = cv[6].x; a[7] = cv[7].x + w00 + w01 + w10 + w11;
        return;
#endif
        const f32x2 W00 = {w00, w00}, W01 = {w01, w01}, W10 = {w10, w10}, W11 = {w11, w11};
        f32x2 r0 = W00 * cv[0].xy, r1 = W00 * cv[0].zw, r2 = W00 * cv[1].xy, r3 = W00 * cv[1].zw;
        r0 += W01 * cv[2].xy; r1 += W01 * cv[2].zw; r2 += W01 * cv[3].xy; r3 += W01 * cv[3].zw;
        r0 += W10 * cv[4].xy; r1 += W10 * cv[4].zw; r2 += W10 * cv[5].xy; r3 += W10 * cv[5].zw;
        r0 += W11 * cv[6].xy; r1 += W11 * cv[6].zw; r2 += W11 * cv[7].xy; r3 += W11 * cv[7].zw;
        a[0] = r0.x; a[1] = r0.y; a[2] = r1.x; a[3] = r1.y; a[4] = r2.x; a[5] = r2.y; a[6] = r3.x; a[7] = r3.y;
    };
    auto mfma_tap = [&](const f32x4 (&bb)[NQ]) {
#ifdef PP_NO_MFMA
        acc[0][0] += a[0] * bb[0].x + a[7] * bb[NQ - 1].w; acc[1][1] += a[3] * bb[1].y + a[5] * bb[0].z; acc[2][0] += a[1]; acc[3][0] += a[2];
        return;
#endif
#define PP_MM(ch, t, wa, av) acc[2 * (ch) + (t)] = __builtin_amdgcn_mfma_f32_16x16x4f32(wa, av, acc[2 * (ch) + (t)], 0, 0, 0);
        if constexpr (CG == 32) {
            PP_MM(0, 0, bb[0].x, a[0]) PP_MM(0, 1, bb[2].x, a[0]) PP_MM(1, 0, bb[0].y, a[1]) PP_MM(1, 1, bb[2].y, a[1])
            PP_MM(0, 0, bb[0].z, a[2]) PP_MM(0, 1, bb[2].z, a[2]) PP_MM(1, 0, bb[0].w, a[3]) PP_MM(1, 1, bb[2].w, a[3])
            PP_MM(0, 0, bb[1].x, a[4]) PP_MM(0, 1, bb[3].x, a[4]) PP_MM(1, 0, bb[1].y, a[5]) PP_MM(1, 1, bb[3].y, a[5])
            PP_MM(0, 0, bb[1].z, a[6]) PP_MM(0, 1, bb[3].z, a[6]) PP_MM(1, 0, bb[1].w, a[7]) PP_MM(1, 1, bb[3].w, a[7])
        } else {
            PP_MM(0, 0, bb[0].x, a[0]) PP_MM(0, 1, bb[1].x, a[4]) PP_MM(1, 0, bb[0].y, a[1]) PP_MM(1, 1, bb[1].y, a[5])
            PP_MM(0, 0, bb[0].z, a[2]) PP_MM(0, 1, bb[1].z, a[6]) PP_MM(1, 0, bb[0].w, a[3]) PP_MM(1, 1, bb[1].w, a[7])
        }
#undef PP_MM
    };

    auto pin_corners = [&]() {
        asm volatile("" : "+v"(cv[0]), "+v"(cv[1]), "+v"(cv[2]), "+v"(cv[3]), "+v"(cv[4]), "+v"(cv[5]), "+v"(cv[6]), "+v"(cv[7]));
    };
    TileXY cur = tile_xy(0), nxt = cur;
    unsigned base_cur = patch_b0, base_nxt = patch_b0 + PATCH_B;
    unsigned tab_cur = tab_b0, tab_nxt = tab_b0 + pp::TAB_B;
    bool have_next = false;
    int it = 0;
    auto tap = [&](auto K, auto FARC) {
        constexpr int k = decltype(K)::value;
        constexpr int kn = (k + 1) % 9;
        if (k == 0) {
            done[0] = acc[0] + acc[2]; done[1] = acc[1] + acc[3];
#pragma unroll
            for (int j = 0; j < 4; ++j) acc[j] = (f32x4){0.f, 0.f, 0.f, 0.f};
        }
        blend();
        prep(k == 8 ? base_nxt : base_cur);
        if constexpr (kn < RW) issue_reads(FARC, kn, b[0], false, k == 8 ? nxt.tn : cur.tn);
        else issue_reads(FARC, kn, b[(k + 1) & 1], true, k == 8 ? nxt.tn : cur.tn);
#ifndef PP_NO_SIDE
#ifndef PP_NO_EPI
        if (k == 0 && it > 0) epilogue();
#endif
        if (k == 1) {
            have_next = it + 1 < n_items;
            if (have_next) {
                nxt = tile_xy(it + 1);
#ifndef PP_NO_DMA
                issue_patch(nxt, base_nxt);
                issue_table(nxt, tab_nxt);
#endif
            }
        }
#endif
        if (k == 7) {
            __builtin_amdgcn_s_waitcnt(0x0070);
            PP_BARRIER();
        }
        read_entry(k >= 7 ? tab_nxt : tab_cur, (kn + 1) % 9);
        PP_SLOT();
        if constexpr (k < RW) mfma_tap(wres[k]);
        else mfma_tap(b[k & 1]);
        PP_SLOT();
        pin_corners();
    };

    __syncthreads();
    read_entry(tab_cur, 0);
    prep(base_cur);
    bool wg_far = true;
    if constexpr ((CG == 16 || PP_SPLIT32) && NT == 2) {
        const unsigned* tflag = reinterpret_cast<const unsigned*>(table + (size_t)ntiles * pp::NE);
        wg_far = false;
        for (int t = t0 + lane; t < t1; t += 64) {
            const TileXY T = tile_of(t);
            wg_far |= tflag[(T.tn * tiles_y + T.ty) * tiles_x + T.tx] != 0u;
        }
        wg_far = __ballot(wg_far) != 0;
    }
    if constexpr (RW > 0) issue_reads(std::true_type{}, 0, b[0], false, cur.tn);
    else issue_reads(std::true_type{}, 0, b[0], true, cur.tn);
    read_entry(tab_cur, 1);
#pragma unroll
    for (int j = 0; j < 4; ++j) acc[j] = (f32x4){0.f, 0.f, 0.f, 0.f};
    auto items = [&](auto FARC) {
        for (it = 0; it < n_items; ++it) {
            tap(std::integral_constant<int, 0>{}, FARC); tap(std::integral_constant<int, 1>{}, FARC); tap(std::integral_constant<int, 2>{}, FARC);
            tap(std::integral_constant<int, 3>{}, FARC); tap(std::integral_constant<int, 4>{}, FARC); tap(std::integral_constant<int, 5>{}, FARC);
            tap(std::integral_constant<int, 6>{}, FARC); tap(std::integral_constant<int, 7>{}, FARC); tap(std::integral_constant<int, 8>{}, FARC);
            prev = cur; prev_valid = tile_valid(it); cur = nxt;
            unsigned tb = base_cur; base_cur = base_nxt; base_nxt = tb;
            tb = tab_cur; tab_cur = tab_nxt; tab_nxt = tb;
        }
    };
    if constexpr ((CG == 16 || PP_SPLIT32) && NT == 2) {
        if (wg_far) items(std::true_type{});
        else items(std::false_type{});
    } else {
        items(std::true_type{});
    }
    done[0] = acc[0] + acc[2]; done[1] = acc[1] + acc[3];
    epilogue();
}

}

static int scratch_table(size_t bytes, hipStream_t stream, void** out) {
    struct Slot { hipStream_t stream; void* buf; size_t cap; };
    static std::mutex mu;
    static std::vector<Slot> slots;
    std::lock_guard<std::mutex> lock(mu);
    Slot* sl = nullptr;
    for (Slot& c : slots) if (c.stream == stream) sl = &c;
    if (!sl) { slots.push_back(Slot{stream, nullptr, 0}); sl = &slots.back(); }
    if (bytes > sl->cap) {
        hipStreamCaptureStatus st = hipStreamCaptureStatusNone;
        (void)hipStreamIsCapturing(stream, &st);
        if (st != hipStreamCaptureStatusNone) {
            wt::set_error("wd_deform_conv3x3: the sampling-table scratch would have to grow, which is not possible inside a stream capture: run "
                          "the shape once eagerly on this stream first, or pass a table (wd_deform_offsets_table_f32)");
            return WT_ERR_INVALID;
        }
        void* fresh = nullptr;
        const size_t want = bytes + bytes / 4;
        WT_HIP(hipMalloc(&fresh, want));
        sl->buf = fresh;
        sl->cap = want;
    }
    *out = sl->buf;
    return WT_OK;
}

int wd_deform_pp_launch(const float* x, const float* offset, const float* packed_weight, const float* scale,
                        const float* bias, int relu, int batch, int h, int w, int c, int cg, int stride, hipStream_t stream, float* y,
                        const void* table) {
    static wt::OncePerDevice attr;
    if (const int dev = wt::device_index(); attr.needed(dev)) {
        WT_HIP(hipFuncSetAttribute(reinterpret_cast<const void*>(deform_conv3x3_pp_kernel<32>),
                                   hipFuncAttributeMaxDynamicSharedMemorySize, (int)pp::smem_bytes<32>()));
        WT_HIP(hipFuncSetAttribute(reinterpret_cast<const void*>(deform_conv3x3_pp_kernel<16>),
                                   hipFuncAttributeMaxDynamicSharedMemorySize, (int)pp::smem_bytes<16>()));
        attr.mark(dev);
    }
    const int ho = (h + 2 - 3) / stride + 1, wo = (w + 2 - 3) / stride + 1;
    const int items = c / pp::CH;
    const int ntiles = batch * ((ho + 7) / 8) * ((wo + 7) / 8);
    if (!table || stride != 1) {
        void* scratch = nullptr;
        WT_TRY(scratch_table(wd_deform_table_bytes(batch, ho, wo), stream, &scratch));
        hipLaunchKernelGGL(deform_table_kernel, dim3((unsigned)(ntiles < 65535 ? ntiles : 65535)), dim3(pp::NE), 0, stream, offset, batch, h, w,
                           ho, wo, stride, (uint4*)scratch);
        WT_HIP(hipGetLastError());
        table = scratch;
    }
    const int n_cu = wt::device_cus() > 0 ? wt::device_cus() : 256;
    int nsplit = n_cu / items;
    if (nsplit < 1) nsplit = 1;
    if (nsplit > (ntiles + pp::NT - 1) / pp::NT) nsplit = (ntiles + pp::NT - 1) / pp::NT;
    if (nsplit < 1) nsplit = 1;
    const float* wfrag = packed_weight + (size_t)c * cg * 9;
    const dim3 grid((unsigned)(items * nsplit));
    if (cg == 32)
        hipLaunchKernelGGL(deform_conv3x3_pp_kernel<32>, grid, dim3(512), pp::smem_bytes<32>(), stream, x, wfrag, scale, bias, relu, batch,
                           h, w, ho, wo, stride, c, c, nsplit, y, (const uint4*)table);
    else
        hipLaunchKernelGGL(deform_conv3x3_pp_kernel<16>, grid, dim3(512), pp::smem_bytes<16>(), stream, x, wfrag, scale, bias, relu, batch,
                           h, w, ho, wo, stride, c, c, nsplit, y, (const uint4*)table);
    WT_HIP(hipGetLastError());
    return WT_OK;
}

extern "C" size_t wd_deform_table_bytes(int batch, int h, int w) {
    const size_t ntiles = (size_t)batch * ((h + 7) / 8) * ((w + 7) / 8);
    return ntiles * pp::TAB_B + (ntiles * 4 + 15) / 16 * 16;
}

extern "C" int wd_deform_offsets_table_f32(const float* partial, int ld, const float* bias, int batch, int h, int w, float* offsets,
                                           void* table, void* stream) {
    WT_TRY(wt::ensure_device());
    if (!partial || !offsets || !table || ld < 162 || (ld & 1) || batch < 1 || h < 1 || w < 1 || ((uintptr_t)partial & 7) ||
        ((uintptr_t)offsets & 7) || ((uintptr_t)table & 15)) {
        wt::set_error("wd_deform_offsets_table_f32: invalid arguments (ld=%d)", ld);
        return WT_ERR_INVALID;
    }
    const long ntiles = (long)batch * ((h + 7) / 8) * ((w + 7) / 8);
    hipLaunchKernelGGL(deform_offsets_table_kernel, dim3((unsigned)(ntiles < 65535 ? ntiles : 65535)), dim3(pp::NE), 0, (hipStream_t)stream,
                       partial, ld, bias, batch, h, w, offsets, (uint4*)table);
    WT_HIP(hipGetLastError());
    return WT_OK;
}
```

Baseline: 44.69 frames/s.

## Add wide 21x21 single-group patch variant for stride-2 deformable conv with 16-channel groups

Adds a templated geometry to the pipelined deformable conv kernel and a new instance for stride-2 layers with 16 channels per group. That instance stages a 21x21 input patch holding one 16-channel group, instead of a 14x14 patch covering two groups. The larger footprint matches the stride-2 sampling window, so fewer bilinear samples should fall outside the LDS patch and take the slow global-memory path. In exchange each work item covers half the channels, so there are more items, and the kernel needs more LDS and a register-limit check at setup.

```diff
diff --git a/include/waymodet.h b/include/waymodet.h
--- a/include/waymodet.h
+++ b/include/waymodet.h
@@ -95,6 +95,7 @@
                               const float* scale, const float* bias, int relu, int batch, int h, int w, int c_in,
                               int c_out, int groups, int stride, int pad, int far_offsets, const void* table, float* y,
                               void* stream);
+int wd_deform_table_f32(const float* offsets, int batch, int h, int w, int c_in, int groups, int stride, void* table, void* stream);
 
 int wd_gemm_nt_f32(const float* A, const float* Bt, const float* bias, const float* residual, int relu,
                    int M, int N, int K, float* C, void* stream);
diff --git a/waymo_2d_tracking_amd/csrc/det_deform.hip b/waymo_2d_tracking_amd/csrc/det_deform.hip
--- a/waymo_2d_tracking_amd/csrc/det_deform.hip
+++ b/waymo_2d_tracking_amd/csrc/det_deform.hip
@@ -666,8 +666,8 @@
 
 
 int wd_deform_pp_launch(const float* x, const float* offset, const float* packed_weight, const float* scale,
-                        const float* bias, int relu, int batch, int h, int w, int c, int cg, int stride, hipStream_t stream, float* y,
-                        const void* table);
+                        const float* bias, int relu, int batch, int h, int w, int c, int cg, int stride, int wide_s2, hipStream_t stream,
+                        float* y, const void* table);
 int wd_grouped_conv3x3_c8_launch(const float* x, const float* packed_weight, const float* scale, const float* bias, int relu,
                                  int batch, int h, int w, int c, hipStream_t stream, float* y);
 
@@ -771,7 +771,8 @@
     if (variant == 3 && stride == 1 && (mask || far_offsets)) variant = 2;
     if (cg == 8 || cg == 16 || cg == 32 || cg == 64) last_kernel = variant_kernel_name(variant, cg, offset != nullptr);
     if (variant == 3)
-        return wd_deform_pp_launch(x, offset, packed_weight, scale, bias, relu, batch, h, w, c_in, cg, stride, stream, y, table);
+        return wd_deform_pp_launch(x, offset, packed_weight, scale, bias, relu, batch, h, w, c_in, cg, stride,
+                                   !(mode && strcmp(mode, "pp14") == 0) && !far_offsets, stream, y, table);
     if (variant == 2) {
         const long nwg_p = ntiles * (c_in / PCH);
         dim3 gridp((unsigned)((nwg_p + 7) / 8 * 8));
diff --git a/waymo_2d_tracking_amd/csrc/det_deform_pp.hip b/waymo_2d_tracking_amd/csrc/det_deform_pp.hip
--- a/waymo_2d_tracking_amd/csrc/det_deform_pp.hip
+++ b/waymo_2d_tracking_amd/csrc/det_deform_pp.hip
@@ -15,11 +15,13 @@
 #define PP_SPLIT32 0
 #endif
 namespace pp {
-constexpr int PS = 14;
-constexpr int NPIX = PS * PS;
-constexpr int CH = 32;
-constexpr int PATCH_F = (NPIX + 1) * CH;
-constexpr int PATCH_B = PATCH_F * 4;
+template <int PS_, int PCH_> struct Geo {
+    static constexpr int PS = PS_, PCH = PCH_;
+    static constexpr int SQ = PCH_ / 4;
+    static constexpr int NPIX = PS_ * PS_;
+    static constexpr int PATCH_F = (NPIX + 1) * PCH_;
+    static constexpr int PATCH_B = PATCH_F * 4;
+};
 constexpr int NE = 64 * 9;
 constexpr int TAB_B = NE * 16;
 constexpr unsigned FAR_Y = 0xFFFFFFFFu;
@@ -27,9 +29,12 @@
 #define PP_RES_TAPS 3
 #endif
 constexpr int RW = PP_RES_TAPS;
-template <int CG> constexpr int tap_floats() { return (CG == 32 ? 4 : 2) * 64 * 4; }
+template <int CG, int PCH> constexpr int nq() { return CG == 32 ? 4 : PCH == 32 ? 2 : 1; }
+template <int CG, int PCH> constexpr int tap_floats() { return nq<CG, PCH>() * 64 * 4; }
 constexpr int NT = 2;
-template <int CG> constexpr size_t smem_bytes() { return (size_t)(9 - RW) * tap_floats<CG>() * 4 + 2 * NT * (size_t)PATCH_B + 2 * NT * (size_t)TAB_B; }
+template <int CG, int PS, int PCH> constexpr size_t smem_bytes() {
+    return (size_t)(9 - RW) * tap_floats<CG, PCH>() * 4 + 2 * NT * (size_t)Geo<PS, PCH>::PATCH_B + 2 * NT * (size_t)TAB_B;
+}
 }
 
 #ifdef PP_NO_BARRIER
@@ -46,18 +51,18 @@
     return y * 8 + x;
 }
 
-__device__ __forceinline__ int pp_slot(int p, int q) { return (p << 3) + (q ^ ((p >> 1) & 7)); }
-
-__device__ __forceinline__ int pp_origin(int stride) { return stride == 1 ? 3 : -1; }
+__device__ __forceinline__ int pp_slot(int p, int q, int sq) { return p * sq + (q ^ ((p >> 1) & (sq - 1))); }
+
+__host__ __device__ __forceinline__ int pp_origin(int stride) { return stride == 1 ? 3 : -1; }
+template <int PS> __host__ __device__ __forceinline__ int pp_patch_origin(int stride) { return PS == 14 ? pp_origin(stride) : 3; }
 
 __device__ __forceinline__ uint4 pp_make_entry(bool pixel_in_image, int yy, int xx, int kh, int kw, float2 ov, int ty, int tx, int H, int W,
-                                               int stride) {
-    constexpr int ps = pp::PS;
-    const int org = pp_origin(stride);
+                                               int stride, int ps, int sq, int porg) {
+    const int org = pp_origin(stride), shift = porg - org;
     const float t_fy = (float)(stride * yy + kh - 1 + org), t_fx = (float)(stride * xx + kw - 1 + org);
     const float py0 = (float)(ty * 8 * stride - org), px0 = (float)(tx * 8 * stride - org);
     const float fH = (float)H, fW = (float)W;
-    unsigned s0 = pp_slot(ps * ps, 0), s1 = s0, s2 = s0, s3 = s0;
+    unsigned s0 = pp_slot(ps * ps, 0, sq), s1 = s0, s2 = s0, s3 = s0;
     float lh = 0.f, lw = 0.f;
     uint4 e;
     if (pixel_in_image) {
@@ -67,9 +72,9 @@
             const float fy = floorf(ry), fx = floorf(rx);
             const int hl = (int)fy, wl = (int)fx;
             lh = ry - fy; lw = rx - fx;
-            if ((unsigned)hl <= (unsigned)(ps - 2) && (unsigned)wl <= (unsigned)(ps - 2)) {
-                const int u = hl * ps + wl;
-                s0 = pp_slot(u, 0); s1 = pp_slot(u + 1, 0); s2 = pp_slot(u + ps, 0); s3 = pp_slot(u + ps + 1, 0);
+            if ((unsigned)(hl + shift) <= (unsigned)(ps - 2) && (unsigned)(wl + shift) <= (unsigned)(ps - 2)) {
+                const int u = (hl + shift) * ps + wl + shift;
+                s0 = pp_slot(u, 0, sq); s1 = pp_slot(u + 1, 0, sq); s2 = pp_slot(u + ps, 0, sq); s3 = pp_slot(u + ps + 1, 0, sq);
             } else {
                 const int ih = hl + ty * 8 * stride - org, iw = wl + tx * 8 * stride - org;
                 e.x = (unsigned)(ih + 32768) | ((unsigned)(iw + 32768) << 16);
@@ -123,14 +128,14 @@
             ov = make_float2(a0, a1);
             *reinterpret_cast<float2*>(offsets + (((size_t)tn * H + oy) * W + ox) * 18 + 2 * k) = ov;
         }
-        const uint4 ent = pp_make_entry(in, yy, xx, kh, kw, ov, ty, tx, H, W, 1);
+        const uint4 ent = pp_make_entry(in, yy, xx, kh, kw, ov, ty, tx, H, W, 1, 14, 8, pp_origin(1));
         table[(size_t)t * pp::NE + e] = ent;
         pp_tile_flag(ent.y == pp::FAR_Y, t, ntiles, table);
     }
 }
 
 __global__ __launch_bounds__(576) void deform_table_kernel(const float* __restrict__ offsets, int batch, int Hin, int Win, int H, int W,
-                                                          int stride, uint4* __restrict__ table) {
+                                                          int stride, int ps, int sq, int porg, uint4* __restrict__ table) {
     const int tiles_x = (W + 7) >> 3, tiles_y = (H + 7) >> 3;
     const int ntiles = batch * tiles_y * tiles_x;
     for (int t = blockIdx.x; t < ntiles; t += gridDim.x) {
@@ -145,27 +150,32 @@
         const bool in = oy < H && ox < W;
         float2 ov = make_float2(0.f, 0.f);
         if (in) ov = *reinterpret_cast<const float2*>(offsets + (((size_t)tn * H + oy) * W + ox) * 18 + 2 * k);
-        const uint4 ent = pp_make_entry(in, yy, xx, kh, kw, ov, ty, tx, Hin, Win, stride);
+        const uint4 ent = pp_make_entry(in, yy, xx, kh, kw, ov, ty, tx, Hin, Win, stride, ps, sq, porg);
         table[(size_t)t * pp::NE + e] = ent;
         pp_tile_flag(ent.y == pp::FAR_Y, t, ntiles, table);
     }
 }
 
-template <int CG>
+template <int CG, int PS, int PCH>
 __global__ __launch_bounds__(256 * pp::NT, pp::NT) __attribute__((amdgpu_waves_per_eu(pp::NT, pp::NT))) void deform_conv3x3_pp_kernel(
     const float* __restrict__ x, const float* __restrict__ wfrag, const float* __restrict__ scale, const float* __restrict__ bias,
     int relu, int batch, int H, int W, int Ho, int Wo, int stride, int C, int Cout, int nsplit, float* __restrict__ y,
     const uint4* __restrict__ table) {
-    static_assert(CG == 32 || CG == 16, "32 channels per group, or two groups of 16 per item");
-    constexpr int NQ = CG == 32 ? 4 : 2;
+    static_assert((CG == 32 && PCH == 32) || (CG == 16 && (PCH == 32 || PCH == 16)), "an item = one group of 32, two groups of 16 or one group of 16");
+    using G = pp::Geo<PS, PCH>;
+    constexpr int NQ = pp::nq<CG, PCH>();
+    constexpr int NQD = PCH / 16;
+    constexpr int OT = PCH / 16;
+    constexpr int SQ = G::SQ;
     constexpr int RW = pp::RW, NT = pp::NT;
-    constexpr int PS = pp::PS, NPIX = pp::NPIX;
-    constexpr int PATCH_F = pp::PATCH_F, PATCH_B = pp::PATCH_B;
-    constexpr int NPC = (NPIX * 8 + 255) / 256;
-    static_assert((NPIX + 1) * 8 * 16 <= 65536, "corner byte offsets are 16 bits");
+    constexpr int NPIX = G::NPIX;
+    constexpr int PATCH_F = G::PATCH_F, PATCH_B = G::PATCH_B;
+    constexpr int NPC = (NPIX * SQ + 255) / 256;
+    static_assert((NPIX + 1) * SQ * 16 <= 65536, "corner byte offsets are 16 bits");
+    static_assert(pp::smem_bytes<CG, PS, PCH>() <= 160 * 1024, "LDS of a CU");
     extern __shared__ __attribute__((aligned(16))) char smem[];
     float* bw = reinterpret_cast<float*>(smem);
-    constexpr unsigned PATCH0 = (unsigned)((9 - RW) * pp::tap_floats<CG>() * 4);
+    constexpr unsigned PATCH0 = (unsigned)((9 - RW) * pp::tap_floats<CG, PCH>() * 4);
     constexpr unsigned TAB0 = PATCH0 + 2u * NT * PATCH_B;
     const int tid = threadIdx.x, lane = tid & 63;
     const int wave = __builtin_amdgcn_readfirstlane(tid >> 6);
@@ -173,7 +183,7 @@
     const int r16 = lane & 15, kq = lane >> 4;
     const int tiles_x = (Wo + 7) >> 3, tiles_y = (Ho + 7) >> 3;
     const int ntiles = batch * tiles_y * tiles_x;
-    const int org = pp_origin(stride), tstep = 8 * stride;
+    const int org = pp_patch_origin<PS>(stride), tstep = 8 * stride;
     const int g = blockIdx.x / nsplit, sidx = blockIdx.x - g * nsplit;
     const int tq = ntiles / nsplit, trm = ntiles - tq * nsplit;
     const int t0 = sidx * tq + (sidx < trm ? sidx : trm);
@@ -181,7 +191,7 @@
     const int n_items = (t1 - t0 + NT - 1) / NT;
     const unsigned patch_b0 = PATCH0 + (unsigned)team * 2u * PATCH_B;
     const unsigned tab_b0 = TAB0 + (unsigned)team * 2u * pp::TAB_B;
-    const int c0 = g * pp::CH;
+    const int c0 = g * PCH;
     const long HW = (long)H * W, HWo = (long)Ho * Wo;
     const char* xb = reinterpret_cast<const char*>(x);
 
@@ -189,10 +199,10 @@
 #pragma unroll
     for (int j = 0; j < NPC; ++j) {
         const int sl = (NPC * m + j) * 64 + lane;
-        const int pxl = sl >> 3, q = (sl & 7) ^ ((pxl >> 1) & 7);
+        const int pxl = sl / SQ, q = (sl & (SQ - 1)) ^ ((pxl >> 1) & (SQ - 1));
         const int r = pxl / PS, cc = pxl - r * PS;
         p_rel[j] = ((r * W + cc) * C + q * 4) * 4;
-        p_rc[j] = (sl < NPIX * 8) ? ((r << 8) | cc) : 0xFFFF;
+        p_rc[j] = (sl < NPIX * SQ) ? ((r << 8) | cc) : 0xFFFF;
     }
 
     struct TileXY { int tn, ty, tx; };
@@ -225,8 +235,8 @@
 #pragma unroll
             for (int j = 0; j < NPC; ++j) {
                 const int s0 = (NPC * m + j) * 64;
-                if (s0 + 64 <= NPIX * 8) dma16(pbase, p_rel[j], base + s0 * 16);
-                else if (s0 < NPIX * 8) { if (p_rc[j] != 0xFFFF) dma16(pbase, p_rel[j], base + s0 * 16); }
+                if (s0 + 64 <= NPIX * SQ) dma16(pbase, p_rel[j], base + s0 * 16);
+                else if (s0 < NPIX * SQ) { if (p_rc[j] != 0xFFFF) dma16(pbase, p_rel[j], base + s0 * 16); }
             }
             return;
         }
@@ -234,7 +244,7 @@
 #pragma unroll
         for (int j = 0; j < NPC; ++j) {
             const int s0 = (NPC * m + j) * 64;
-            if (s0 >= NPIX * 8) continue;
+            if (s0 >= NPIX * SQ) continue;
             const int iy = py0 + (p_rc[j] >> 8), ix = px0 + (p_rc[j] & 255);
             const bool in = p_rc[j] != 0xFFFF && iy >= 0 && iy < H && ix >= 0 && ix < W;
             if (in) {
@@ -259,7 +269,7 @@
     };
 
     f32x4 wres[RW > 0 ? RW : 1][NQ];
-    float4 aff_sc[2], aff_bi[2];
+    float4 aff_sc[OT], aff_bi[OT];
     {
         if constexpr (CG == 32) {
             const f32x4* src = reinterpret_cast<const f32x4*>(wfrag + (size_t)g * 9 * 64 * 16);
@@ -271,6 +281,11 @@
             for (int k = 0; k < RW; ++k)
 #pragma unroll
                 for (int j = 0; j < NQ; ++j) wres[k][j] = src[(k * 64 + lane) * 4 + j];
+        } else if constexpr (PCH == 16) {
+            const f32x4* src = reinterpret_cast<const f32x4*>(wfrag + (size_t)g * 9 * 64 * 4);
+            for (int e = tid; e < (9 - RW) * 64; e += 256 * NT) *reinterpret_cast<f32x4*>(bw + e * 4) = src[e + RW * 64];
+#pragma unroll
+            for (int k = 0; k < RW; ++k) wres[k][0] = src[k * 64 + lane];
         } else {
             const f32x4* src = reinterpret_cast<const f32x4*>(wfrag + (size_t)(2 * g) * 9 * 64 * 4);
             for (int e = tid; e < (9 - RW) * 2 * 64; e += 256 * NT) {
@@ -283,19 +298,19 @@
                 for (int j = 0; j < NQ; ++j) wres[k][j] = src[(j * 9 + k) * 64 + lane];
         }
 #pragma unroll
-        for (int nt = 0; nt < 2; ++nt) {
+        for (int nt = 0; nt < OT; ++nt) {
             const int c = c0 + 16 * nt + 4 * kq;
             aff_sc[nt] = scale ? *reinterpret_cast<const float4*>(scale + c) : make_float4(1.f, 1.f, 1.f, 1.f);
             aff_bi[nt] = bias ? *reinterpret_cast<const float4*>(bias + c) : make_float4(0.f, 0.f, 0.f, 0.f);
         }
-        if (tid < 2 * NT * pp::CH)
-            reinterpret_cast<float*>(smem + PATCH0)[(tid >> 5) * PATCH_F + NPIX * pp::CH + (tid & 31)] = 0.f;
+        if (tid < 2 * NT * PCH)
+            reinterpret_cast<float*>(smem + PATCH0)[(tid / PCH) * PATCH_F + NPIX * PCH + (tid % PCH)] = 0.f;
         const TileXY T0 = tile_xy(0);
         issue_patch(T0, patch_b0);
         issue_table(T0, tab_b0);
         __builtin_amdgcn_s_waitcnt(0x0F70);
     }
-    f32x4 acc[4], done[2];
+    f32x4 acc[4], done[OT];
     const int my_p = pp_row_pixel(r16, m);
     const int my_y = my_p >> 3, my_x = my_p & 7;
 
@@ -307,7 +322,7 @@
         if (ho < Ho && wo < Wo) {
             float* dst = y + ((long)prev.tn * HWo + (long)ho * Wo + wo) * Cout + c0 + 4 * kq;
 #pragma unroll
-            for (int nt = 0; nt < 2; ++nt) {
+            for (int nt = 0; nt < OT; ++nt) {
                 const float4 sc = aff_sc[nt], bi = aff_bi[nt];
                 float4 v;
                 v.x = done[nt][0] * sc.x + bi.x; v.y = done[nt][1] * sc.y + bi.y;
@@ -318,9 +333,9 @@
         }
     };
 
-    float a[8];
+    float a[4 * NQD];
     f32x4 b[2][NQ];
-    f32x4 cv[8];
+    f32x4 cv[4 * NQD];
     float w00 = 0.f, w01 = 0.f, w10 = 0.f, w11 = 0.f;
     bool far_nxt = false;
     unsigned ad0 = 0, ad1 = 0, ad2 = 0, ad3 = 0;
@@ -347,10 +362,14 @@
 #endif
     };
     auto lds_corners = [&]() {
-        cv[0] = *(lds4)(uintptr_t)ad0; cv[1] = *(lds4)(uintptr_t)(ad0 ^ QX);
-        cv[2] = *(lds4)(uintptr_t)ad1; cv[3] = *(lds4)(uintptr_t)(ad1 ^ QX);
-        cv[4] = *(lds4)(uintptr_t)ad2; cv[5] = *(lds4)(uintptr_t)(ad2 ^ QX);
-        cv[6] = *(lds4)(uintptr_t)ad3; cv[7] = *(lds4)(uintptr_t)(ad3 ^ QX);
+        if constexpr (NQD == 2) {
+            cv[0] = *(lds4)(uintptr_t)ad0; cv[1] = *(lds4)(uintptr_t)(ad0 ^ QX);
+            cv[2] = *(lds4)(uintptr_t)ad1; cv[3] = *(lds4)(uintptr_t)(ad1 ^ QX);
+            cv[4] = *(lds4)(uintptr_t)ad2; cv[5] = *(lds4)(uintptr_t)(ad2 ^ QX);
+            cv[6] = *(lds4)(uintptr_t)ad3; cv[7] = *(lds4)(uintptr_t)(ad3 ^ QX);
+        } else {
+            cv[0] = *(lds4)(uintptr_t)ad0; cv[1] = *(lds4)(uintptr_t)ad1; cv[2] = *(lds4)(uintptr_t)ad2; cv[3] = *(lds4)(uintptr_t)ad3;
+        }
     };
     auto issue_reads = [&](auto FARC, int k, f32x4 (&bb)[NQ], bool want_w, int tn) {
         constexpr bool FAR = decltype(FARC)::value;
@@ -367,10 +386,15 @@
                 const unsigned ch_b = (unsigned)my_ch * 4u, rowa = (unsigned)(ya * W), rowb = (unsigned)(yb * W), cb = (unsigned)C * 4u;
                 const unsigned o00 = (rowa + (unsigned)xa) * cb + ch_b, o01 = (rowa + (unsigned)xc) * cb + ch_b;
                 const unsigned o10 = (rowb + (unsigned)xa) * cb + ch_b, o11 = (rowb + (unsigned)xc) * cb + ch_b;
-                cv[0] = *reinterpret_cast<const f32x4*>(gb + o00); cv[1] = *reinterpret_cast<const f32x4*>(gb + (o00 + Q2));
-                cv[2] = *reinterpret_cast<const f32x4*>(gb + o01); cv[3] = *reinterpret_cast<const f32x4*>(gb + (o01 + Q2));
-                cv[4] = *reinterpret_cast<const f32x4*>(gb + o10); cv[5] = *reinterpret_cast<const f32x4*>(gb + (o10 + Q2));
-                cv[6] = *reinterpret_cast<const f32x4*>(gb + o11); cv[7] = *reinterpret_cast<const f32x4*>(gb + (o11 + Q2));
+                if constexpr (NQD == 2) {
+                    cv[0] = *reinterpret_cast<const f32x4*>(gb + o00); cv[1] = *reinterpret_cast<const f32x4*>(gb + (o00 + Q2));
+                    cv[2] = *reinterpret_cast<const f32x4*>(gb + o01); cv[3] = *reinterpret_cast<const f32x4*>(gb + (o01 + Q2));
+                    cv[4] = *reinterpret_cast<const f32x4*>(gb + o10); cv[5] = *reinterpret_cast<const f32x4*>(gb + (o10 + Q2));
+                    cv[6] = *reinterpret_cast<const f32x4*>(gb + o11); cv[7] = *reinterpret_cast<const f32x4*>(gb + (o11 + Q2));
+                } else {
+                    cv[0] = *reinterpret_cast<const f32x4*>(gb + o00); cv[1] = *reinterpret_cast<const f32x4*>(gb + o01);
+                    cv[2] = *reinterpret_cast<const f32x4*>(gb + o10); cv[3] = *reinterpret_cast<const f32x4*>(gb + o11);
+                }
             } else {
                 lds_corners();
             }
@@ -386,19 +410,29 @@
     };
     auto blend = [&]() {
 #ifdef PP_NO_BLEND
-        a[0] = cv[0].x; a[1] = cv[1].y; a[2] = cv[2].x; a[3] = cv[3].y; a[4] = cv[4].x; a[5] = cv[5].x; a[6] = cv[6].x; a[7] = cv[7].x + w00 + w01 + w10 + w11;
+        if constexpr (NQD == 2) { a[4] = cv[4].x; a[5] = cv[5].x; a[6] = cv[6].x; a[7] = cv[7].x; }
+        a[0] = cv[0].x; a[1] = cv[1].y; a[2] = cv[2].x; a[3] = cv[3].y + w00 + w01 + w10 + w11;
         return;
 #endif
         const f32x2 W00 = {w00, w00}, W01 = {w01, w01}, W10 = {w10, w10}, W11 = {w11, w11};
+        if constexpr (NQD == 1) {
+            f32x2 r0 = W00 * cv[0].xy, r1 = W00 * cv[0].zw;
+            r0 += W01 * cv[1].xy; r1 += W01 * cv[1].zw;
+            r0 += W10 * cv[2].xy; r1 += W10 * cv[2].zw;
+            r0 += W11 * cv[3].xy; r1 += W11 * cv[3].zw;
+            a[0] = r0.x; a[1] = r0.y; a[2] = r1.x; a[3] = r1.y;
+            return;
+        } else {
         f32x2 r0 = W00 * cv[0].xy, r1 = W00 * cv[0].zw, r2 = W00 * cv[1].xy, r3 = W00 * cv[1].zw;
         r0 += W01 * cv[2].xy; r1 += W01 * cv[2].zw; r2 += W01 * cv[3].xy; r3 += W01 * cv[3].zw;
         r0 += W10 * cv[4].xy; r1 += W10 * cv[4].zw; r2 += W10 * cv[5].xy; r3 += W10 * cv[5].zw;
         r0 += W11 * cv[6].xy; r1 += W11 * cv[6].zw; r2 += W11 * cv[7].xy; r3 += W11 * cv[7].zw;
         a[0] = r0.x; a[1] = r0.y; a[2] = r1.x; a[3] = r1.y; a[4] = r2.x; a[5] = r2.y; a[6] = r3.x; a[7] = r3.y;
+        }
     };
     auto mfma_tap = [&](const f32x4 (&bb)[NQ]) {
 #ifdef PP_NO_MFMA
-        acc[0][0] += a[0] * bb[0].x + a[7] * bb[NQ - 1].w; acc[1][1] += a[3] * bb[1].y + a[5] * bb[0].z; acc[2][0] += a[1]; acc[3][0] += a[2];
+        acc[0][0] += a[0] * bb[0].x + a[4 * NQD - 1] * bb[NQ - 1].w; acc[1][1] += a[3] * bb[NQ - 1].y + a[4 * NQD - 3] * bb[0].z; acc[2][0] += a[1]; acc[3][0] += a[2];
         return;
 #endif
 #define PP_MM(ch, t, wa, av) acc[2 * (ch) + (t)] = __builtin_amdgcn_mfma_f32_16x16x4f32(wa, av, acc[2 * (ch) + (t)], 0, 0, 0);
@@ -407,6 +441,8 @@
             PP_MM(0, 0, bb[0].z, a[2]) PP_MM(0, 1, bb[2].z, a[2]) PP_MM(1, 0, bb[0].w, a[3]) PP_MM(1, 1, bb[2].w, a[3])
             PP_MM(0, 0, bb[1].x, a[4]) PP_MM(0, 1, bb[3].x, a[4]) PP_MM(1, 0, bb[1].y, a[5]) PP_MM(1, 1, bb[3].y, a[5])
             PP_MM(0, 0, bb[1].z, a[6]) PP_MM(0, 1, bb[3].z, a[6]) PP_MM(1, 0, bb[1].w, a[7]) PP_MM(1, 1, bb[3].w, a[7])
+        } else if constexpr (PCH == 16) {
+            PP_MM(0, 0, bb[0].x, a[0]) PP_MM(1, 0, bb[0].y, a[1]) PP_MM(0, 0, bb[0].z, a[2]) PP_MM(1, 0, bb[0].w, a[3])
         } else {
             PP_MM(0, 0, bb[0].x, a[0]) PP_MM(0, 1, bb[1].x, a[4]) PP_MM(1, 0, bb[0].y, a[1]) PP_MM(1, 1, bb[1].y, a[5])
             PP_MM(0, 0, bb[0].z, a[2]) PP_MM(0, 1, bb[1].z, a[6]) PP_MM(1, 0, bb[0].w, a[3]) PP_MM(1, 1, bb[1].w, a[7])
@@ -415,7 +451,8 @@
     };
 
     auto pin_corners = [&]() {
-        asm volatile("" : "+v"(cv[0]), "+v"(cv[1]), "+v"(cv[2]), "+v"(cv[3]), "+v"(cv[4]), "+v"(cv[5]), "+v"(cv[6]), "+v"(cv[7]));
+        if constexpr (NQD == 2) asm volatile("" : "+v"(cv[0]), "+v"(cv[1]), "+v"(cv[2]), "+v"(cv[3]), "+v"(cv[4]), "+v"(cv[5]), "+v"(cv[6]), "+v"(cv[7]));
+        else asm volatile("" : "+v"(cv[0]), "+v"(cv[1]), "+v"(cv[2]), "+v"(cv[3]));
     };
     TileXY cur = tile_xy(0), nxt = cur;
     unsigned base_cur = patch_b0, base_nxt = patch_b0 + PATCH_B;
@@ -426,7 +463,8 @@
         constexpr int k = decltype(K)::value;
         constexpr int kn = (k + 1) % 9;
         if (k == 0) {
-            done[0] = acc[0] + acc[2]; done[1] = acc[1] + acc[3];
+            done[0] = acc[0] + acc[2];
+            if constexpr (OT == 2) done[1] = acc[1] + acc[3];
 #pragma unroll
             for (int j = 0; j < 4; ++j) acc[j] = (f32x4){0.f, 0.f, 0.f, 0.f};
         }
@@ -495,7 +533,8 @@
     } else {
         items(std::true_type{});
     }
-    done[0] = acc[0] + acc[2]; done[1] = acc[1] + acc[3];
+    done[0] = acc[0] + acc[2];
+    if constexpr (OT == 2) done[1] = acc[1] + acc[3];
     epilogue();
 }
 
@@ -527,25 +566,16 @@
     return WT_OK;
 }
 
-int wd_deform_pp_launch(const float* x, const float* offset, const float* packed_weight, const float* scale,
-                        const float* bias, int relu, int batch, int h, int w, int c, int cg, int stride, hipStream_t stream, float* y,
-                        const void* table) {
-    static wt::OncePerDevice attr;
-    if (const int dev = wt::device_index(); attr.needed(dev)) {
-        WT_HIP(hipFuncSetAttribute(reinterpret_cast<const void*>(deform_conv3x3_pp_kernel<32>),
-                                   hipFuncAttributeMaxDynamicSharedMemorySize, (int)pp::smem_bytes<32>()));
-        WT_HIP(hipFuncSetAttribute(reinterpret_cast<const void*>(deform_conv3x3_pp_kernel<16>),
-                                   hipFuncAttributeMaxDynamicSharedMemorySize, (int)pp::smem_bytes<16>()));
-        attr.mark(dev);
-    }
-    const int ho = (h + 2 - 3) / stride + 1, wo = (w + 2 - 3) / stride + 1;
-    const int items = c / pp::CH;
+template <int CG, int PS, int PCH>
+static int pp_launch_instance(const float* x, const float* offset, const float* wfrag, const float* scale, const float* bias, int relu, int batch,
+                              int h, int w, int ho, int wo, int c, int stride, hipStream_t stream, float* y, const void* table) {
+    const int items = c / PCH;
     const int ntiles = batch * ((ho + 7) / 8) * ((wo + 7) / 8);
     if (!table || stride != 1) {
         void* scratch = nullptr;
         WT_TRY(scratch_table(wd_deform_table_bytes(batch, ho, wo), stream, &scratch));
         hipLaunchKernelGGL(deform_table_kernel, dim3((unsigned)(ntiles < 65535 ? ntiles : 65535)), dim3(pp::NE), 0, stream, offset, batch, h, w,
-                           ho, wo, stride, (uint4*)scratch);
+                           ho, wo, stride, PS, pp::Geo<PS, PCH>::SQ, pp_patch_origin<PS>(stride), (uint4*)scratch);
         WT_HIP(hipGetLastError());
         table = scratch;
     }
@@ -554,14 +584,61 @@
     if (nsplit < 1) nsplit = 1;
     if (nsplit > (ntiles + pp::NT - 1) / pp::NT) nsplit = (ntiles + pp::NT - 1) / pp::NT;
     if (nsplit < 1) nsplit = 1;
+    const dim3 grid((unsigned)(items * nsplit));
+    constexpr size_t smem = pp::smem_bytes<CG, PS, PCH>();
+    hipLaunchKernelGGL((deform_conv3x3_pp_kernel<CG, PS, PCH>), grid, dim3(512), smem, stream, x, wfrag, scale, bias,
+                       relu, batch, h, w, ho, wo, stride, c, c, nsplit, y, (const uint4*)table);
+    WT_HIP(hipGetLastError());
+    return WT_OK;
+}
+
+template <int CG, int PS, int PCH> static int pp_prepare_instance(int max_regs) {
+    const void* fn = reinterpret_cast<const void*>(deform_conv3x3_pp_kernel<CG, PS, PCH>);
+    WT_HIP(hipFuncSetAttribute(fn, hipFuncAttributeMaxDynamicSharedMemorySize, (int)pp::smem_bytes<CG, PS, PCH>()));
+    hipFuncAttributes at{};
+    WT_HIP(hipFuncGetAttributes(&at, fn));
+    if (at.numRegs > max_regs) {
+        wt::set_error("deform_conv3x3_pp_kernel<%d, %d, %d>: %d VGPRs (limit %d)", CG, PS, PCH, at.numRegs, max_regs);
+        return WT_ERR_INVALID;
+    }
+    return WT_OK;
+}
+
+int wd_deform_pp_launch(const float* x, const float* offset, const float* packed_weight, const float* scale,
+                        const float* bias, int relu, int batch, int h, int w, int c, int cg, int stride, int wide_s2, hipStream_t stream,
+                        float* y, const void* table) {
+    static wt::OncePerDevice attr;
+    if (const int dev = wt::device_index(); attr.needed(dev)) {
+        WT_TRY((pp_prepare_instance<32, 14, 32>(256)));
+        WT_TRY((pp_prepare_instance<16, 14, 32>(256)));
+        WT_TRY((pp_prepare_instance<16, 21, 16>(192)));
+        attr.mark(dev);
+    }
+    const int ho = (h + 2 - 3) / stride + 1, wo = (w + 2 - 3) / stride + 1;
     const float* wfrag = packed_weight + (size_t)c * cg * 9;
-    const dim3 grid((unsigned)(items * nsplit));
     if (cg == 32)
-        hipLaunchKernelGGL(deform_conv3x3_pp_kernel<32>, grid, dim3(512), pp::smem_bytes<32>(), stream, x, wfrag, scale, bias, relu, batch,
-                           h, w, ho, wo, stride, c, c, nsplit, y, (const uint4*)table);
-    else
-        hipLaunchKernelGGL(deform_conv3x3_pp_kernel<16>, grid, dim3(512), pp::smem_bytes<16>(), stream, x, wfrag, scale, bias, relu, batch,
-                           h, w, ho, wo, stride, c, c, nsplit, y, (const uint4*)table);
+        return pp_launch_instance<32, 14, 32>(x, offset, wfrag, scale, bias, relu, batch, h, w, ho, wo, c, stride, stream, y, table);
+    if (stride == 2 && wide_s2)
+        return pp_launch_instance<16, 21, 16>(x, offset, wfrag, scale, bias, relu, batch, h, w, ho, wo, c, stride, stream, y, table);
+    return pp_launch_instance<16, 14, 32>(x, offset, wfrag, scale, bias, relu, batch, h, w, ho, wo, c, stride, stream, y, table);
+}
+
+extern "C" int wd_deform_table_f32(const float* offsets, int batch, int h, int w, int c_in, int groups, int stride, void* table,
+                                   void* stream) {
+    WT_TRY(wt::ensure_device());
+    const int cg = (groups > 0 && c_in > 0 && c_in % groups == 0) ? c_in / groups : 0;
+    if (!offsets || !table || batch < 1 || h < 1 || w < 1 || (cg != 16 && cg != 32) || (stride != 1 && stride != 2) ||
+        ((uintptr_t)offsets & 7) || ((uintptr_t)table & 15)) {
+        wt::set_error("wd_deform_table_f32: invalid arguments (c_in=%d groups=%d stride=%d)", c_in, groups, stride);
+        return WT_ERR_INVALID;
+    }
+    const int ho = (h + 2 - 3) / stride + 1, wo = (w + 2 - 3) / stride + 1;
+    if (ho < 1 || wo < 1) return WT_OK;
+    const bool wide = stride == 2 && cg == 16;
+    const int ps = wide ? 21 : 14, sq = wide ? 4 : 8, org = wide ? pp_patch_origin<21>(stride) : pp_patch_origin<14>(stride);
+    const long ntiles = (long)batch * ((ho + 7) / 8) * ((wo + 7) / 8);
+    hipLaunchKernelGGL(deform_table_kernel, dim3((unsigned)(ntiles < 65535 ? ntiles : 65535)), dim3(pp::NE), 0, (hipStream_t)stream, offsets,
+                       batch, h, w, ho, wo, stride, ps, sq, org, (uint4*)table);
     WT_HIP(hipGetLastError());
     return WT_OK;
 }
```

Result: no change. 44.74 frames/s (median of 2 runs) (+0.1%).
